# aleflabo/PREGO

Measured on AMD Instinct MI355X. Metric: frames/sec (per-frame action logits) on Assembly101-O TSN features, higher is better.
Workload: dtype fp16; 1 GPU; BASELINE configs[1]: Assembly101-O-test-split-shaped eval set, MiniROAD eval path (rgb+flow fp32 [T,2048] each -> per-frame probs[86] + argmax); clips_per_gpu=182, frames_per_gpu=2306143, min_T=3342, max_T=33981, flow=non-zero (full K=4096 layer1 GEMM), parallelism=clip-sharded dp1, no collective: every rank its own eval-set-sized clip list, weights=random init, seed 20

## Files before the change

### include/prego_amd_debug.h

```cpp
#ifndef PREGO_AMD_DEBUG_H
#define PREGO_AMD_DEBUG_H
#include "prego_amd.h"
#ifdef __cplusplus
extern "C" {
#endif

int prego_debug_head_only(prego_miniroad* h, int n_slots, int n_steps, const void* h_relu, float* out, int32_t* argmax,
                          const void* rowmap , prego_stream_t stream);

int prego_miniroad_debug_stamps(prego_miniroad* h, unsigned long long* out8);

int prego_debug_recurrence_only(prego_miniroad* h, int n_slots, int n_steps, int gd, const void* gi, void* h_relu, prego_stream_t stream);
int prego_debug_gemm_worker(const void* A, const void* B, const float* bias, float* C, int M, int N, int K, int xcd_lo,
                            unsigned* counter, int grid, prego_stream_t stream);

int prego_debug_split_fault(prego_miniroad* h, int mode);
int prego_debug_split_state(const prego_miniroad* h, int64_t* fallbacks, int32_t* fails, int64_t* skip, int32_t* split_env);
int prego_debug_set_abort(prego_miniroad* h, unsigned value, prego_stream_t stream);
int prego_debug_alloc_count(int64_t* device_mallocs, int64_t* host_waits);
int prego_debug_ant_full_span(int on);
int prego_debug_hog(int kind, int xcd_lo, int ms, const void* read_buf, void* write_buf, size_t bytes, float* sink, prego_stream_t stream);

int prego_debug_gemm_bf16(int variant, const void* A, const void* B, const float* bias, float* C, int M, int N, int K,
                          prego_stream_t stream);

int prego_debug_gemm_tn(int ta, int tb, const void* A, int lda, const void* B, int ldb, const float* bias, float* C, void* C16, int ldc,
                        int M, int N, int K, int k_valid, float* colsum_out, prego_stream_t stream);

int prego_debug_gemm_nt(int f16, int train_splitk, const void* A, int lda, const void* B, int ldb, const float* bias, float* C, int ldc,
                        int M, int N, int K, prego_stream_t stream);

int prego_debug_attention_bwd(int batch, int len, int heads, int dh, int causal, const void* qs, const void* k, const void* v,
                              const void* o, const void* dout, const float* lse, void* dqkv, prego_stream_t stream);

int prego_debug_attention_fwd(int batch, int n_query, int len, int heads, int dh, int causal, const void* qs, const void* k,
                              const void* v, void* out, float* lse, prego_stream_t stream);

#ifdef __cplusplus
}
#endif
#endif
```

### prego_amd/_lib.py

```python
from __future__ import annotations

import ctypes as C
import os

_HERE = os.path.dirname(os.path.abspath(__file__))
DEBUG_LIB_PATH = os.path.join(_HERE, "lib", "libprego_amd_debug.so")
LIB_PATH = os.environ.get("PREGO_AMD_LIB") or (DEBUG_LIB_PATH if os.environ.get("PREGO_AMD_DEBUG_LIB") else os.path.join(_HERE, "lib", "libprego_amd.so"))

PREGO_F32, PREGO_BF16, PREGO_F16, PREGO_F16X2 = 0, 1, 2, 3
FWD_SOFTMAX, FWD_KEEP, FWD_IN16 = 1, 2, 4
E_TIMEOUT = -4

SYMBOLS = [
    "prego_abi_version", "prego_last_error",
    "prego_miniroad_create", "prego_miniroad_create_layers", "prego_miniroad_set_gru_layer", "prego_miniroad_destroy", "prego_miniroad_last_error", "prego_miniroad_set_weights",
    "prego_miniroad_max_clips", "prego_miniroad_workspace_bytes", "prego_miniroad_forward",
    "prego_miniroad_check", "prego_miniroad_timing_enable", "prego_miniroad_timing_read",
    "prego_miniroad_set_dropout", "prego_oad_loss", "prego_oad_loss_reduce",
    "prego_miniroad_backward_workspace_bytes", "prego_miniroad_backward", "prego_adamw_step", "prego_miniroad_adamw_step", "prego_window_vote", "prego_format_ids", "prego_perframe_ap_labels", "prego_onehot_labels",
    "prego_vit_create", "prego_vit_destroy", "prego_vit_num_tensors", "prego_vit_set_weights",
    "prego_vit_workspace_bytes", "prego_vit_forward",
    "prego_vit_set_dropout", "prego_vit_train_workspace_bytes", "prego_vit_forward_train", "prego_vit_backward",
    "prego_attention_layer_workspace_bytes", "prego_attention_layer_forward",
    "prego_attention_layer_create", "prego_attention_layer_destroy", "prego_attention_layer_set_weights",
    "prego_attention_layer_handle_workspace_bytes", "prego_attention_layer_handle_forward",
    "prego_attention_layer_set_dropout", "prego_attention_layer_train_workspace_bytes", "prego_attention_layer_forward_train", "prego_attention_layer_backward", "prego_vit_adamw_step", "prego_miniroad_step",
    "prego_perframe_ap_workspace_bytes", "prego_perframe_ap", "prego_vit_frames_workspace_bytes", "prego_vit_forward_frames", "prego_miniroad_backward_events", "prego_miniroad_backward_callback",
    "prego_miniroad_plan_starts", "prego_miniroad_set_feed_events", "prego_miniroad_pass_info",
    "prego_vit_set_compute_dtype", "prego_attention_layer_set_compute_dtype",
    "prego_miniroad_resident_bytes", "prego_miniroad_set_resident", "prego_miniroad_guard_publish", "prego_miniroad_set_peer_guard",
    "prego_miniroad_set_gru_layer_grads",
    "prego_miniroad_set_anticipation", "prego_miniroad_forward_anticipation",
    "prego_miniroad_set_anticipation_grads", "prego_miniroad_adamw_step_anticipation",
    "prego_miniroad_step_anticipation",
    "prego_miniroad_step_wide_workspace_bytes", "prego_miniroad_step_wide", "prego_miniroad_step_wide_anticipation",
    "prego_cast_features",
    "prego_stream_pool_bytes", "prego_stream_pool_create", "prego_stream_pool_destroy", "prego_miniroad_step_pool_workspace_bytes",
    "prego_miniroad_step_pool", "prego_stream_pool_vote", "prego_stream_pool_flush", "prego_stream_pool_reset", "prego_stream_pool_record",
    "prego_miniroad_step_frames_workspace_bytes", "prego_miniroad_step_frames", "prego_miniroad_step_frames_anticipation",
    "prego_miniroad_step_pool_frames_workspace_bytes", "prego_miniroad_step_pool_frames",
    "prego_miniroad_step_ragged_workspace_bytes", "prego_miniroad_step_ragged", "prego_miniroad_step_ragged_anticipation",
    "prego_miniroad_step_pool_ragged_workspace_bytes", "prego_miniroad_step_pool_ragged",
]
DEBUG_SYMBOLS = ["prego_miniroad_debug_stamps", "prego_debug_gemm_bf16", "prego_debug_attention_bwd", "prego_debug_attention_fwd",
                 "prego_debug_recurrence_only", "prego_debug_gemm_worker", "prego_debug_head_only",
                 "prego_debug_split_fault", "prego_debug_split_state", "prego_debug_set_abort", "prego_debug_alloc_count", "prego_debug_hog",
                 "prego_debug_ant_full_span", "prego_debug_gemm_tn", "prego_debug_gemm_nt"]


class PregoError(RuntimeError):
    pass


_lib = None


def _open(path: str, debug: bool) -> C.CDLL:
    if not os.path.exists(path):
        raise PregoError(
            f"{path} not found: the HIP library has not been built. Run `python -m prego_amd.build` "
            "(needs hipcc; cross-compiles gfx950 without a GPU). There is no CPU fallback.")
    import torch
    lib = C.CDLL(path)
    vp, i32, i64, sz = C.c_void_p, C.c_int, C.c_int64, C.c_size_t
    lib.prego_abi_version.restype = i32
    lib.prego_last_error.restype = C.c_char_p
    lib.prego_miniroad_create.argtypes = [C.POINTER(vp), i32, i32, i32, i32, i32, i32]
    lib.prego_miniroad_create_layers.argtypes = [C.POINTER(vp), i32, i32, i32, i32, i32, i32, i32]
    lib.prego_miniroad_set_gru_layer.argtypes = [vp, i32, vp, vp, vp, vp, vp]
    lib.prego_miniroad_destroy.argtypes = [vp]
    lib.prego_miniroad_destroy.restype = None
    lib.prego_miniroad_last_error.argtypes = [vp]
    lib.prego_miniroad_last_error.restype = C.c_char_p
    lib.prego_miniroad_set_weights.argtypes = [vp] + [vp] * 10 + [vp]
    lib.prego_miniroad_max_clips.argtypes = [vp]
    lib.prego_miniroad_workspace_bytes.argtypes = [vp, i32, C.POINTER(C.c_int32), i64, i32]
    lib.prego_miniroad_workspace_bytes.restype = sz
    lib.prego_miniroad_resident_bytes.argtypes = [vp, i32, C.POINTER(C.c_int32), i32]
    lib.prego_miniroad_resident_bytes.restype = sz
    lib.prego_miniroad_set_resident.argtypes = [vp, vp, sz]
    lib.prego_miniroad_guard_publish.argtypes = [vp, vp, vp]
    lib.prego_miniroad_set_peer_guard.argtypes = [vp, vp]
    lib.prego_miniroad_set_gru_layer_grads.argtypes = [vp, i32, vp, vp, vp, vp]
    lib.prego_miniroad_forward.argtypes = [vp, i32, C.POINTER(C.c_int32), C.POINTER(vp), C.POINTER(vp),
                                           C.POINTER(vp), C.POINTER(vp), vp, vp, i32, vp, sz, vp]
    lib.prego_miniroad_set_anticipation.argtypes = [vp, i32, vp, vp, vp]
    lib.prego_miniroad_forward_anticipation.argtypes = [vp, i32, C.POINTER(C.c_int32), C.POINTER(vp), C.POINTER(vp),
                                                        C.POINTER(vp), C.POINTER(vp), C.POINTER(vp), C.POINTER(vp), vp, vp, i32, vp, sz, vp]
    lib.prego_miniroad_set_anticipation_grads.argtypes = [vp, C.POINTER(vp), vp, vp]
    lib.prego_miniroad_step.argtypes = [vp, i32, vp, vp, vp, vp, vp, i32, vp]
    lib.prego_miniroad_step_anticipation.argtypes = [vp, i32, vp, vp, vp, vp, vp, vp, vp, i32, vp]
    lib.prego_miniroad_step_wide_workspace_bytes.argtypes = [vp, i32]
    lib.prego_miniroad_step_wide_workspace_bytes.restype = sz
    lib.prego_miniroad_step_wide.argtypes = [vp, i32, vp, vp, vp, vp, vp, i32, vp, sz, vp]
    lib.prego_miniroad_step_wide_anticipation.argtypes = [vp, i32, vp, vp, vp, vp, vp, vp, vp, i32, vp, sz, vp]
    lib.prego_stream_pool_bytes.argtypes = [vp, i32, i32]
    lib.prego_stream_pool_bytes.restype = sz
    lib.prego_stream_pool_create.argtypes = [C.POINTER(vp), vp, i32, i32, i32, vp, sz, vp]
    lib.prego_stream_pool_destroy.argtypes = [vp]
    lib.prego_stream_pool_destroy.restype = None
    lib.prego_miniroad_step_pool_workspace_bytes.argtypes = [vp, i32]
    lib.prego_miniroad_step_pool_workspace_bytes.restype = sz
    lib.prego_miniroad_step_pool.argtypes = [vp, vp, i32, C.POINTER(C.c_int32), vp, vp, vp, vp, vp, vp, i32, vp, sz, vp]
    lib.prego_miniroad_step_frames_workspace_bytes.argtypes = [vp, i32, i32]
    lib.prego_miniroad_step_frames_workspace_bytes.restype = sz
    lib.prego_miniroad_step_frames.argtypes = [vp, i32, i32, vp, vp, vp, vp, vp, i32, vp, sz, vp]
    lib.prego_miniroad_step_frames_anticipation.argtypes = [vp, i32, i32, vp, vp, vp, vp, vp, vp, vp, i32, vp, sz, vp]
    lib.prego_miniroad_step_pool_frames_workspace_bytes.argtypes = [vp, i32, i32]
    lib.prego_miniroad_step_pool_frames_workspace_bytes.restype = sz
    lib.prego_miniroad_step_pool_frames.argtypes = [vp, vp, i32, i32, C.POINTER(C.c_int32), vp, vp, vp, vp, vp, vp, i32, vp, sz, vp]
    lib.prego_miniroad_step_ragged_workspace_bytes.argtypes = [vp, i32, i32]
    lib.prego_miniroad_step_ragged_workspace_bytes.restype = sz
    lib.prego_miniroad_step_ragged.argtypes = [vp, i32, C.POINTER(C.c_int32), vp, vp, vp, vp, vp, i32, vp, sz, vp]
    lib.prego_miniroad_step_ragged_anticipation.argtypes = [vp, i32, C.POINTER(C.c_int32), vp, vp, vp, vp, vp, vp, vp, i32, vp, sz, vp]
    lib.prego_miniroad_step_pool_ragged_workspace_bytes.argtypes = [vp, i32, i32]
    lib.prego_miniroad_step_pool_ragged_workspace_bytes.restype = sz
    lib.prego_miniroad_step_pool_ragged.argtypes = [vp, vp, i32, C.POINTER(C.c_int32), C.POINTER(C.c_int32), vp, vp, vp, vp, vp, vp, i32, vp, sz,
                                                    vp]
    lib.prego_stream_pool_vote.argtypes = [vp, i32, C.POINTER(C.c_int32), vp, vp]
    lib.prego_stream_pool_flush.argtypes = [vp, i32, C.POINTER(C.c_int32), vp]
    lib.prego_stream_pool_reset.argtypes = [vp, i32, C.POINTER(C.c_int32), vp]
    lib.prego_stream_pool_record.argtypes = [vp, i32, C.POINTER(vp), C.POINTER(sz)]
    lib.prego_miniroad_check.argtypes = [vp, vp]
    lib.prego_miniroad_timing_enable.argtypes = [vp, i32]
    lib.prego_miniroad_timing_read.argtypes = [vp, C.POINTER(C.c_double), C.POINTER(i64), C.POINTER(C.c_double),
                                               C.POINTER(C.c_double), C.POINTER(i64), C.POINTER(C.c_double),
                                               C.POINTER(i64), C.POINTER(C.c_double)]
    lib.prego_miniroad_set_dropout.argtypes = [vp, C.c_float, C.c_uint64]
    lib.prego_oad_loss.argtypes = [i32, C.POINTER(C.c_int32), C.POINTER(vp), C.POINTER(vp), i32, vp, C.POINTER(vp),
                                   C.c_float, vp]
    lib.prego_oad_loss_reduce.argtypes = [i32, C.POINTER(C.c_int32), C.POINTER(vp), C.POINTER(vp), i32, i32, vp, C.POINTER(vp),
                                          C.c_float, vp]
    lib.prego_miniroad_backward_workspace_bytes.argtypes = [vp, i32, C.POINTER(C.c_int32)]
    lib.prego_miniroad_backward_workspace_bytes.restype = sz
    lib.prego_miniroad_backward.argtypes = [vp, i32, C.POINTER(C.c_int32), C.POINTER(vp)] + [vp] * 10 + [vp, sz, vp, sz, vp]
    lib.prego_miniroad_backward_events.argtypes = [vp, vp, vp]
    lib.prego_miniroad_backward_callback.argtypes = [vp, vp, vp]
    lib.prego_miniroad_plan_starts.argtypes = [vp, i32, C.POINTER(C.c_int32), i32, C.POINTER(C.c_int32), C.POINTER(C.c_int32)]
    lib.prego_miniroad_set_feed_events.argtypes = [vp, i32, C.POINTER(C.c_int32), C.POINTER(vp), i32]
    lib.prego_miniroad_pass_info.argtypes = [vp, C.POINTER(C.c_int32), C.POINTER(C.c_int32), C.POINTER(C.c_int32)]
    lib.prego_window_vote.argtypes = [vp, i64, i32, i32, vp, vp]
    lib.prego_format_ids.argtypes = [vp, i64, vp, vp, vp]
    lib.prego_cast_features.argtypes = [vp, vp, i64, i32, vp]
    lib.prego_perframe_ap_workspace_bytes.argtypes = [i64, i32]
    lib.prego_perframe_ap_workspace_bytes.restype = sz
    lib.prego_perframe_ap.argtypes = [vp, vp, i64, i32, vp, vp, vp, vp, sz, vp]
    lib.prego_perframe_ap_labels.argtypes = [vp, vp, i64, i32, vp, vp, vp, vp, sz, vp]
    lib.prego_onehot_labels.argtypes = [i32, C.POINTER(vp), C.POINTER(i64), i32, vp, C.POINTER(C.c_int32)]
    f32 = C.c_float
    lib.prego_adamw_step.argtypes = [i32, C.POINTER(vp), C.POINTER(vp), C.POINTER(vp), C.POINTER(vp), C.POINTER(i64), i64, f32, f32, f32, f32, f32, vp]
    lib.prego_miniroad_adamw_step.argtypes = [vp, C.POINTER(vp), C.POINTER(vp), C.POINTER(vp), C.POINTER(vp), i64, f32, f32, f32, f32, f32, vp]
    lib.prego_miniroad_adamw_step_anticipation.argtypes = [vp, C.POINTER(vp), C.POINTER(vp), C.POINTER(vp), C.POINTER(vp), i64, f32, f32, f32, f32, f32, vp]
    lib.prego_vit_adamw_step.argtypes = [vp, C.POINTER(vp), C.POINTER(vp), C.POINTER(vp), C.POINTER(vp), i32, i64, f32, f32, f32, f32, f32, vp]
    lib.prego_vit_create.argtypes = [C.POINTER(vp)] + [i32] * 8
    lib.prego_vit_destroy.argtypes = [vp]
    lib.prego_vit_destroy.restype = None
    lib.prego_vit_num_tensors.argtypes = [vp]
    lib.prego_vit_set_weights.argtypes = [vp, C.POINTER(vp), i32, vp]
    lib.prego_vit_workspace_bytes.argtypes = [vp, i32]
    lib.prego_vit_workspace_bytes.restype = sz
    lib.prego_vit_forward.argtypes = [vp, i32, vp, vp, vp, i32, vp, sz, vp]
    lib.prego_vit_frames_workspace_bytes.argtypes = [vp, i32, i32]
    lib.prego_vit_frames_workspace_bytes.restype = sz
    lib.prego_vit_forward_frames.argtypes = [vp, i32, vp, vp, vp, vp, i32, i32, vp, sz, vp]
    lib.prego_vit_set_compute_dtype.argtypes = [vp, i32]
    lib.prego_attention_layer_set_compute_dtype.argtypes = [vp, i32]
    lib.prego_vit_set_dropout.argtypes = [vp, C.c_float, C.c_float, C.c_uint64]
    lib.prego_vit_train_workspace_bytes.argtypes = [vp, i32]
    lib.prego_vit_train_workspace_bytes.restype = sz
    lib.prego_vit_forward_train.argtypes = [vp, i32, vp, vp, vp, i32, vp, sz, vp]
    lib.prego_vit_backward.argtypes = [vp, i32, vp, C.POINTER(vp), i32, i32, vp, sz, vp]
    lib.prego_attention_layer_workspace_bytes.argtypes = [i32, i32, i32]
    lib.prego_attention_layer_workspace_bytes.restype = sz
    lib.prego_attention_layer_forward.argtypes = [i32] * 5 + [vp] * 10 + [vp, sz, vp]
    lib.prego_attention_layer_create.argtypes = [C.POINTER(vp), i32, i32]
    lib.prego_attention_layer_destroy.argtypes = [vp]
    lib.prego_attention_layer_destroy.restype = None
    lib.prego_attention_layer_set_weights.argtypes = [vp] + [vp] * 8 + [vp]
    lib.prego_attention_layer_handle_workspace_bytes.argtypes = [vp, i32, i32]
    lib.prego_attention_layer_handle_workspace_bytes.restype = sz
    lib.prego_attention_layer_handle_forward.argtypes = [vp, i32, i32, i32, vp, vp, vp, sz, vp]
    lib.prego_attention_layer_set_dropout.argtypes = [vp, C.c_float, C.c_uint64]
    lib.prego_attention_layer_train_workspace_bytes.argtypes = [vp, i32, i32]
    lib.prego_attention_layer_train_workspace_bytes.restype = sz
    lib.prego_attention_layer_forward_train.argtypes = [vp, i32, i32, i32, vp, vp, vp, sz, vp]
    lib.prego_attention_layer_backward.argtypes = [vp, i32, i32, i32, vp, vp, vp, i32, vp, sz, vp]
    for name in SYMBOLS:
        getattr(lib, name)
    if debug:
        lib.prego_miniroad_debug_stamps.argtypes = [vp, C.POINTER(C.c_uint64)]
        lib.prego_debug_head_only.argtypes = [vp, i32, i32, vp, vp, vp, vp, vp]
        lib.prego_debug_attention_bwd.argtypes = [i32] * 5 + [vp] * 7 + [vp]
        lib.prego_debug_attention_fwd.argtypes = [i32] * 6 + [vp] * 5 + [vp]
        lib.prego_debug_recurrence_only.argtypes = [vp, i32, i32, i32, vp, vp, vp]
        lib.prego_debug_gemm_worker.argtypes = [vp, vp, vp, vp, i32, i32, i32, i32, vp, i32, vp]
        lib.prego_debug_gemm_bf16.argtypes = [i32, vp, vp, vp, vp, i32, i32, i32, vp]
        lib.prego_debug_gemm_tn.argtypes = [i32, i32, vp, i32, vp, i32, vp, vp, vp, i32, i32, i32, i32, i32, vp, vp]
        lib.prego_debug_gemm_nt.argtypes = [i32, i32, vp, i32, vp, i32, vp, vp, i32, i32, i32, i32, vp]
        lib.prego_debug_split_fault.argtypes = [vp, i32]
        lib.prego_debug_split_state.argtypes = [vp, C.POINTER(i64), C.POINTER(i32), C.POINTER(i64), C.POINTER(i32)]
        lib.prego_debug_set_abort.argtypes = [vp, C.c_uint32, vp]
        lib.prego_debug_alloc_count.argtypes = [C.POINTER(i64), C.POINTER(i64)]
        lib.prego_debug_hog.argtypes = [i32, i32, i32, vp, vp, sz, vp, vp]
        lib.prego_debug_ant_full_span.argtypes = [i32]
    return lib


def load() -> C.CDLL:
    global _lib
    if _lib is None:
        _lib = _open(LIB_PATH, debug=LIB_PATH == DEBUG_LIB_PATH)
    return _lib


_dbg = None


def load_debug() -> C.CDLL:
    global _dbg
    if _dbg is None:
        _dbg = load() if LIB_PATH == DEBUG_LIB_PATH else _open(DEBUG_LIB_PATH, debug=True)
    return _dbg




def check(rc: int):
    if rc != 0:
        raise PregoError(f"prego_amd error {rc}: {load().prego_last_error().decode()}")


def ptr_array(ptrs):
    arr = (C.c_void_p * len(ptrs))()
    for i, p in enumerate(ptrs):
        arr[i] = p
    return arr
```

### prego_amd/csrc/ff_pass.hip

```cpp
#include "common.h"
#include "kernels.h"
#include "pass_handshake.h"

#define FBK 64
#define FHALF 16384
#define FBUF 65536
#define FF_WAIT(n) asm volatile("s_waitcnt vmcnt(" #n ")" ::: "memory")
#define FF_TIMEOUT_TICKS 200000000ull

__device__ __forceinline__ int ffp_key_b(int r) { return ((r >> 1) & 1) | (((r >> 3) & 3) << 1); }

__device__ __forceinline__ bool ffp_wait_ge(const unsigned* p, unsigned need, unsigned* abort_word, unsigned code) {
  if (__hip_atomic_load(p, __ATOMIC_RELAXED, __HIP_MEMORY_SCOPE_AGENT) >= need) return true;
  const unsigned long long t0 = __builtin_amdgcn_s_memrealtime();
  unsigned spins = 0;
  for (;;) {
    __builtin_amdgcn_s_sleep(8);
    if (__hip_atomic_load(p, __ATOMIC_RELAXED, __HIP_MEMORY_SCOPE_AGENT) >= need) return true;
    if ((++spins & 31u) == 0u) {
      if (__hip_atomic_load(abort_word, __ATOMIC_RELAXED, __HIP_MEMORY_SCOPE_AGENT)) return false;
      if (__builtin_amdgcn_s_memrealtime() - t0 > FF_TIMEOUT_TICKS) {
        __hip_atomic_store(abort_word, code, __ATOMIC_RELAXED, __HIP_MEMORY_SCOPE_AGENT);
        return false;
      }
    }
  }
}

template <typename OT, bool SC1OUT>
__device__ __forceinline__ void ffp_tile(char* smem, const bf16_t* __restrict__ A, int lda, int rows, const bf16_t* __restrict__ B, int ldb,
                                         const float* __restrict__ bias, bf16_t* __restrict__ C, int ldc, int K) {
  int tid = threadIdx.x;
  asm volatile("" : "+v"(tid));
  const int lane = tid & 63;
  const int wave = __builtin_amdgcn_readfirstlane(tid >> 6);
  const int grp = wave >> 2, wc = wave & 3;
  const int nk = K / FBK;
  const int sr = lane >> 3, scp = lane & 7;
  int a_off[2], b_off[2];
#pragma unroll
  for (int i = 0; i < 2; ++i) {
    const int r = (wave * 2 + i) * 8 + sr;
    a_off[i] = r * lda * 2 + ((scp ^ ((r >> 1) & 7)) << 4);
    b_off[i] = r * ldb * 2 + ((scp ^ ffp_key_b(r)) << 4);
  }
  const __amdgpu_buffer_rsrc_t rs_a = __builtin_amdgcn_make_buffer_rsrc((void*)A, 0, rows * lda * 2, 0x00020000);
  const __amdgpu_buffer_rsrc_t rs_b = __builtin_amdgcn_make_buffer_rsrc((void*)B, 0, 256 * ldb * 2, 0x00020000);
  auto stage_a = [&](int hf, int kt) {
    char* dst = smem + (kt & 1) * FBUF + hf * FHALF + wave * 2048;
    const int so = hf * 128 * lda * 2 + kt * (FBK * 2);
#pragma unroll
    for (int i = 0; i < 2; ++i)
      __builtin_amdgcn_raw_ptr_buffer_load_lds(rs_a, (__attribute__((address_space(3))) void*)(dst + i * 1024), 16, a_off[i], so, 0, 0);
  };
  auto stage_b = [&](int hf, int kt) {
    char* dst = smem + (kt & 1) * FBUF + (2 + hf) * FHALF + wave * 2048;
    const int so = hf * 128 * ldb * 2 + kt * (FBK * 2);
#pragma unroll
    for (int i = 0; i < 2; ++i)
      __builtin_amdgcn_raw_ptr_buffer_load_lds(rs_b, (__attribute__((address_space(3))) void*)(dst + i * 1024), 16, b_off[i], so, 0, 0);
  };
  const int fr = lane & 15, fq = lane >> 4;
  bf16x8 a0[2][4], a1[2][4], b0[2][2], b1[2][2];
  auto read_a = [&](bf16x8 (&af)[2][4], int slot, int kt) {
    const char* base = smem + (kt & 1) * FBUF + slot * FHALF;
#pragma unroll
    for (int ks = 0; ks < 2; ++ks)
#pragma unroll
      for (int i = 0; i < 4; ++i) {
        const int r = grp * 64 + i * 16 + fr;
        af[ks][i] = *(const bf16x8*)(base + r * 128 + (((ks * 4 + fq) ^ ((r >> 1) & 7)) << 4));
      }
  };
  auto read_b = [&](bf16x8 (&bf)[2][2], int slot, int kt) {
    const char* base = smem + (kt & 1) * FBUF + slot * FHALF;
#pragma unroll
    for (int ks = 0; ks < 2; ++ks)
#pragma unroll
      for (int j = 0; j < 2; ++j) {
        const int r = wc * 32 + (fr >> 2) * 8 + j * 4 + (fr & 3);
        bf[ks][j] = *(const bf16x8*)(base + r * 128 + (((ks * 4 + fq) ^ ffp_key_b(r)) << 4));
      }
  };
  f32x4 acc[2][2][4][2];
#pragma unroll
  for (int x = 0; x < 2; ++x)
#pragma unroll
    for (int y = 0; y < 2; ++y)
#pragma unroll
      for (int i = 0; i < 4; ++i)
#pragma unroll
        for (int j = 0; j < 2; ++j) acc[x][y][i][j] = (f32x4){0.f, 0.f, 0.f, 0.f};
  auto mma = [&](f32x4 (&c)[4][2], const bf16x8 (&af)[2][4], const bf16x8 (&bf)[2][2]) {
    asm volatile("s_waitcnt lgkmcnt(0)" ::: "memory");
    __builtin_amdgcn_sched_barrier(0);
    __builtin_amdgcn_s_setprio(1);
#pragma unroll
    for (int ks = 0; ks < 2; ++ks)
#pragma unroll
      for (int i = 0; i < 4; ++i)
#pragma unroll
        for (int j = 0; j < 2; ++j) c[i][j] = op16<OT>::mfma(bf[ks][j], af[ks][i], c[i][j]);
    __builtin_amdgcn_s_setprio(0);
    __builtin_amdgcn_sched_barrier(0);
  };
  auto bar = [&]() {
    __builtin_amdgcn_sched_barrier(0);
    __builtin_amdgcn_s_barrier();
    __builtin_amdgcn_sched_barrier(0);
  };
  stage_a(0, 0); stage_b(0, 0); stage_b(1, 0); stage_a(1, 0);
  stage_a(0, 1); stage_b(0, 1); stage_b(1, 1);
  FF_WAIT(10);
  bar();
  read_a(a0, 0, 0);
  if (grp == 1) bar();
  for (int kt = 0; kt < nk; ++kt) {
    const bool full = kt + 2 < nk;
    read_b(b0, 2, kt);
    if (kt + 1 < nk) stage_a(1, kt + 1);
    if (full) FF_WAIT(10); else FF_WAIT(0);
    bar();
    mma(acc[0][0], a0, b0);
    bar();
    read_b(b1, 3, kt);
    if (full) { stage_a(0, kt + 2); FF_WAIT(10); } else FF_WAIT(0);
    bar();
    mma(acc[0][1], a0, b1);
    bar();
    read_a(a1, 1, kt);
    if (full) { stage_b(0, kt + 2); FF_WAIT(10); } else FF_WAIT(0);
    bar();
    mma(acc[1][1], a1, b1);
    bar();
    if (kt + 1 < nk) read_a(a0, 0, kt + 1);
    if (full) { stage_b(1, kt + 2); FF_WAIT(10); } else FF_WAIT(0);
    bar();
    mma(acc[1][0], a1, b0);
    bar();
  }
  if (grp == 0) bar();
  float4 bv[2][2];
#pragma unroll
  for (int y = 0; y < 2; ++y)
#pragma unroll
    for (int j = 0; j < 2; ++j) bv[y][j] = *(const float4*)(bias + y * 128 + wc * 32 + fq * 8 + j * 4);
  const __amdgpu_buffer_rsrc_t rs_c = __builtin_amdgcn_make_buffer_rsrc((void*)C, 0, rows * ldc * 2, 0x00020000);
#pragma unroll
  for (int x = 0; x < 2; ++x)
#pragma unroll
    for (int y = 0; y < 2; ++y) {
      const int n = y * 128 + wc * 32 + fq * 8;
#pragma unroll
      for (int i = 0; i < 4; ++i) {
        const int m = x * 128 + grp * 64 + i * 16 + fr;
        const f32x4 v0 = acc[x][y][i][0], v1 = acc[x][y][i][1];
        u32x4 pk;
        pk[0] = op16<OT>::pack2_sat(v0[0] + bv[y][0].x, v0[1] + bv[y][0].y); pk[1] = op16<OT>::pack2_sat(v0[2] + bv[y][0].z, v0[3] + bv[y][0].w);
        pk[2] = op16<OT>::pack2_sat(v1[0] + bv[y][1].x, v1[1] + bv[y][1].y); pk[3] = op16<OT>::pack2_sat(v1[2] + bv[y][1].z, v1[3] + bv[y][1].w);
        if constexpr (SC1OUT) __builtin_amdgcn_raw_buffer_store_b128(pk, rs_c, (m * ldc + n) * 2, 0, AUX_SC1);
        else __builtin_amdgcn_raw_buffer_store_b128(pk, rs_c, (m * ldc + n) * 2, 0, 0);
      }
    }
}

template <typename OT, bool IN16>
__device__ __forceinline__ void ffp_pack_rows(const FfPassArgs& a, int my_rows, int wave, int lane, const char* srgb, const char* sflow,
                                              bf16_t* __restrict__ Xs) {
  constexpr int ES = IN16 ? 2 : 4, NV = IN16 ? 1 : 2;
  constexpr int PR = 2;
  const int din = a.kx;
  const int cr_rgb = (a.d_rgb + 2047) >> 11, cpr = cr_rgb + ((a.d_flow + 2047) >> 11);
  const int n_rounds = my_rows > 0 ? ((my_rows + PR - 1) / PR) * cpr : 0;
  auto readlane_ptr = [](const char* p, int l) -> const char* {
    const unsigned long long v = (unsigned long long)p;
    const unsigned lo = (unsigned)__builtin_amdgcn_readlane((int)(unsigned)v, l), hi = (unsigned)__builtin_amdgcn_readlane((int)(unsigned)(v >> 32), l);
    return (const char*)(((unsigned long long)hi << 32) | lo);
  };
  int voff_in = lane * 8 * ES, voff_in2 = voff_in + 1024 * ES, voff_out = lane * 16;
  asm volatile("" : "+v"(voff_in), "+v"(voff_in2), "+v"(voff_out));
  auto issue = [&](u32x4 (&v)[PR][4][NV], int k) {
    const int rp = k / cpr, cj = k - rp * cpr;
    const bool fl = cj >= cr_rgb;
    const int cwin = (fl ? cj - cr_rgb : cj) << 11, seg_len = fl ? a.d_flow : a.d_rgb;
#pragma unroll
    for (int e = 0; e < PR; ++e) {
      const int r = rp * PR + e, rr = r < my_rows ? r : 0;
      const char* s0 = readlane_ptr(srgb, rr);
      const char* s1 = readlane_ptr(sflow, rr);
      const char* src = fl ? s1 : s0;
      const __amdgpu_buffer_rsrc_t rs = __builtin_amdgcn_make_buffer_rsrc((void*)(src + (size_t)cwin * ES), 0,
                                                                          (r < my_rows && src != nullptr) ? (seg_len - cwin) * ES : 0, 0x00020000);
#pragma unroll
      for (int b = 0; b < 4; ++b)
#pragma unroll
        for (int w = 0; w < NV; ++w)
          v[e][b][w] = __builtin_amdgcn_raw_buffer_load_b128(rs, (b < 2 ? voff_in : voff_in2) + ((b & 1) * 512 * ES + 16 * w), 0, AUX_NT);
    }
  };
  auto drain = [&](const u32x4 (&v)[PR][4][NV], int k) {
    const int rp = k / cpr, cj = k - rp * cpr;
    const bool fl = cj >= cr_rgb;
    const int cwin = (fl ? cj - cr_rgb : cj) << 11, seg_len = fl ? a.d_flow : a.d_rgb, seg_base = fl ? a.d_rgb : 0;
#pragma unroll
    for (int e = 0; e < PR; ++e) {
      const int r = rp * PR + e;
      bf16_t* dst = Xs + (size_t)(wave * 32 + (r < my_rows ? r : 0)) * din + seg_base + cwin;
      const __amdgpu_buffer_rsrc_t rs = __builtin_amdgcn_make_buffer_rsrc((void*)dst, 0, r < my_rows ? (seg_len - cwin) * 2 : 0, 0x00020000);
#pragma unroll
      for (int b = 0; b < 4; ++b) {
        u32x4 o = v[e][b][0];
        if constexpr (!IN16) {
          const u32x4 x = v[e][b][0], y = v[e][b][NV - 1];
          o[0] = op16<OT>::pack2_sat(__uint_as_float(x[0]), __uint_as_float(x[1])); o[1] = op16<OT>::pack2_sat(__uint_as_float(x[2]), __uint_as_float(x[3]));
          o[2] = op16<OT>::pack2_sat(__uint_as_float(y[0]), __uint_as_float(y[1])); o[3] = op16<OT>::pack2_sat(__uint_as_float(y[2]), __uint_as_float(y[3]));
        }
        __builtin_amdgcn_raw_buffer_store_b128(o, rs, voff_out + b * 1024, 0, 0);
      }
    }
  };
  u32x4 va[PR][4][NV], vb[PR][4][NV];
  if (n_rounds == 0) return;
  issue(va, 0);
  int k = 0;
#define PACK_FENCE() __builtin_amdgcn_sched_barrier(0)
  for (; k + 2 < n_rounds; k += 2) {
    issue(vb, k + 1); PACK_FENCE();
    drain(va, k); PACK_FENCE();
    issue(va, k + 2); PACK_FENCE();
    drain(vb, k + 1); PACK_FENCE();
  }
  if (k + 1 < n_rounds) {
    issue(vb, k + 1); PACK_FENCE();
    drain(va, k); PACK_FENCE();
    drain(vb, k + 1);
  } else {
    drain(va, k);
  }
#undef PACK_FENCE
}

template <typename OT>
__device__ __forceinline__ void ffp_pack(const FfPassArgs& a, int row0, int nrows, bf16_t* __restrict__ Xs) {
  int tid_ = threadIdx.x;
  asm volatile("" : "+v"(tid_));
  const int lane = tid_ & 63, wave = __builtin_amdgcn_readfirstlane(tid_ >> 6);
  const int rl = wave * 32 + (lane & 31);
  int clip = 0, t = 0;
  if (rl < nrows) {
    const int row = row0 + rl;
    int lo = a.plan.blk_step[row >> 5];
    while (lo + 1 < a.plan.s_max && a.plan.rowoff[lo + 1] <= row) ++lo;
    const int slot = row - a.plan.rowoff[lo];
    int k = a.plan.seg_off[slot];
    const int kend = a.plan.seg_off[slot + 1];
    while (k + 1 < kend && a.plan.seg_start[k + 1] <= lo) ++k;
    clip = a.plan.seg_clip[k];
    t = lo - a.plan.seg_start[k];
    if (a.rowmap != nullptr && lane < 32) ((int2*)a.rowmap)[row] = make_int2(clip, t);
  }
  const char* srgb = nullptr; const char* sflow = nullptr;
  const int es = a.in16 ? 2 : 4;
  if (rl < nrows) {
    const float* rgb = a.rgb_ptrs ? a.rgb_ptrs[clip] : nullptr;
    const float* flow = a.flow_ptrs ? a.flow_ptrs[clip] : nullptr;
    if (rgb) srgb = (const char*)rgb + (size_t)t * a.d_rgb * es;
    if (flow) sflow = (const char*)flow + (size_t)t * a.d_flow * es;
  }
  const int my_rows = nrows - wave * 32 < 32 ? nrows - wave * 32 : 32;
  if (a.in16) ffp_pack_rows<OT, true>(a, my_rows, wave, lane, srgb, sflow, Xs);
  else ffp_pack_rows<OT, false>(a, my_rows, wave, lane, srgb, sflow, Xs);
}

constexpr int FLN_MAX_E = 2048;

template <typename OT, int NV, int NR>
__device__ __forceinline__ void ffp_ln(const FfPassArgs& a, int nrows, const bf16_t* __restrict__ Ys, bf16_t* __restrict__ Es, const float* gb) {
  int tid_ = threadIdx.x;
  asm volatile("" : "+v"(tid_));
  const int lane = tid_ & 63, wave = __builtin_amdgcn_readfirstlane(tid_ >> 6);
  const int E = NV * 512;
  const float fE = (float)a.E;
  if (wave >= nrows) return;
  auto request = [&](u32x4 (&dst)[NR][NV], int rb) {
#pragma unroll
    for (int e = 0; e < NR; ++e) {
      int r = rb + 8 * e;
      if (r >= nrows) r = wave;
      const bf16_t* y = Ys + (size_t)r * E;
#pragma unroll
      for (int i = 0; i < NV; ++i) dst[e][i] = *(const u32x4*)(y + (i * 64 + lane) * 8);
    }
  };
  auto unpack = [](const u32x4 w, float (&f)[8]) {
    f[0] = op16<OT>::lo(w[0]); f[1] = op16<OT>::hi(w[0]); f[2] = op16<OT>::lo(w[1]); f[3] = op16<OT>::hi(w[1]);
    f[4] = op16<OT>::lo(w[2]); f[5] = op16<OT>::hi(w[2]); f[6] = op16<OT>::lo(w[3]); f[7] = op16<OT>::hi(w[3]);
  };
  auto process = [&](const u32x4 (&raw)[NR][NV], int rb) {
    float s[NR];
#pragma unroll
    for (int e = 0; e < NR; ++e) {
      s[e] = 0.f;
#pragma unroll
      for (int i = 0; i < NV; ++i) {
        float f[8];
        unpack(raw[e][i], f);
        s[e] += ((f[0] + f[1]) + (f[2] + f[3])) + ((f[4] + f[5]) + (f[6] + f[7]));
      }
    }
    auto wave_sum_rows = [](float (&v)[NR]) {
#pragma unroll
      for (int o = 32; o > 0; o >>= 1) {
        float t[NR];
#pragma unroll
        for (int e = 0; e < NR; ++e) t[e] = __shfl_xor(v[e], o, 64);
#pragma unroll
        for (int e = 0; e < NR; ++e) v[e] += t[e];
      }
    };
    float mu[NR], rstd[NR];
    wave_sum_rows(s);
#pragma unroll
    for (int e = 0; e < NR; ++e) mu[e] = s[e] / fE;
#pragma unroll
    for (int e = 0; e < NR; ++e) {
      float qq = 0.f;
#pragma unroll
      for (int i = 0; i < NV; ++i) {
        float f[8];
        unpack(raw[e][i], f);
#pragma unroll
        for (int k = 0; k < 8; ++k) {
#pragma clang fp contract(off)
          const float d = f[k] - mu[e];
          const float dd = d * d;
          qq = qq + dd;
        }
      }
      rstd[e] = qq;
    }
    wave_sum_rows(rstd);
#pragma unroll
    for (int e = 0; e < NR; ++e) rstd[e] = 1.0f / sqrtf(rstd[e] / fE + a.ln_eps);
#pragma unroll
    for (int i = 0; i < NV; ++i) {
      const int c = (i * 64 + lane) * 8;
      const float4 g0 = *(const float4*)(gb + c), g1 = *(const float4*)(gb + c + 4);
      const float4 b0 = *(const float4*)(gb + FLN_MAX_E + c), b1 = *(const float4*)(gb + FLN_MAX_E + c + 4);
      const float gg[8] = {g0.x, g0.y, g0.z, g0.w, g1.x, g1.y, g1.z, g1.w};
      const float bb[8] = {b0.x, b0.y, b0.z, b0.w, b1.x, b1.y, b1.z, b1.w};
#pragma unroll
      for (int e = 0; e < NR; ++e) {
        float f[8], o[8];
        unpack(raw[e][i], f);
#pragma unroll
        for (int k = 0; k < 8; ++k) o[k] = fmaxf((f[k] - mu[e]) * rstd[e] * gg[k] + bb[k], 0.f);
        uint4 w;
        w.x = op16<OT>::pack2_sat(o[0], o[1]); w.y = op16<OT>::pack2_sat(o[2], o[3]); w.z = op16<OT>::pack2_sat(o[4], o[5]); w.w = op16<OT>::pack2_sat(o[6], o[7]);
        if (rb + 8 * e < nrows) *(uint4*)(Es + (size_t)(rb + 8 * e) * E + c) = w;
      }
    }
  };
  constexpr int STEP = 8 * NR;
#define LN_FENCE() __builtin_amdgcn_sched_barrier(0)
  u32x4 ra[NR][NV], rbuf[NR][NV];
  int rb = wave;
  request(ra, rb); LN_FENCE();
  for (; rb + 2 * STEP < nrows; rb += 2 * STEP) {
    request(rbuf, rb + STEP); LN_FENCE();
    process(ra, rb); LN_FENCE();
    request(ra, rb + 2 * STEP); LN_FENCE();
    process(rbuf, rb + STEP); LN_FENCE();
  }
  if (rb + STEP < nrows) {
    request(rbuf, rb + STEP); LN_FENCE();
    process(ra, rb); LN_FENCE();
    process(rbuf, rb + STEP);
  } else {
    process(ra, rb);
  }
#undef LN_FENCE
}

template <typename OT, int MAXV, int NR>
__device__ __forceinline__ void ffp_ln_generic(const FfPassArgs& a, int nrows, const bf16_t* __restrict__ Ys, bf16_t* __restrict__ Es) {
  int tid_ = threadIdx.x;
  asm volatile("" : "+v"(tid_));
  const int lane = tid_ & 63, wave = tid_ >> 6;
  const int E = a.E, nv = E / 512;
  u32x4 raw[NR][MAXV], nxt[NR][MAXV];
  auto request = [&](u32x4 (&dst)[NR][MAXV], int rb) {
#pragma unroll
    for (int e = 0; e < NR; ++e) {
      int r = rb + 8 * e;
      if (r >= nrows) r = wave < nrows ? wave : 0;
      const bf16_t* y = Ys + (size_t)r * E;
#pragma unroll
      for (int i = 0; i < MAXV; ++i)
        if (i < nv) dst[e][i] = *(const u32x4*)(y + (i * 64 + lane) * 8);
    }
  };
  if (wave < nrows) request(raw, wave);
  for (int rb = wave; rb < nrows; rb += 8 * NR) {
    if (rb + 8 * NR < nrows) request(nxt, rb + 8 * NR);
    auto unpack = [](const u32x4 w, float (&f)[8]) {
      f[0] = op16<OT>::lo(w[0]); f[1] = op16<OT>::hi(w[0]); f[2] = op16<OT>::lo(w[1]); f[3] = op16<OT>::hi(w[1]);
      f[4] = op16<OT>::lo(w[2]); f[5] = op16<OT>::hi(w[2]); f[6] = op16<OT>::lo(w[3]); f[7] = op16<OT>::hi(w[3]);
    };
    float s[NR];
#pragma unroll
    for (int e = 0; e < NR; ++e) {
      s[e] = 0.f;
#pragma unroll
      for (int i = 0; i < MAXV; ++i)
        if (i < nv) {
          float f[8];
          unpack(raw[e][i], f);
          s[e] += ((f[0] + f[1]) + (f[2] + f[3])) + ((f[4] + f[5]) + (f[6] + f[7]));
        }
    }
    float mu[NR], rstd[NR];
#pragma unroll
    for (int e = 0; e < NR; ++e) mu[e] = wave_sum(s[e]) / (float)E;
#pragma unroll
    for (int e = 0; e < NR; ++e) {
      float qq = 0.f;
#pragma unroll
      for (int i = 0; i < MAXV; ++i)
        if (i < nv) {
          float f[8];
          unpack(raw[e][i], f);
#pragma unroll
          for (int k = 0; k < 8; ++k) {
#pragma clang fp contract(off)
            const float d = f[k] - mu[e];
            const float dd = d * d;
            qq = qq + dd;
          }
        }
      rstd[e] = qq;
    }
#pragma unroll
    for (int e = 0; e < NR; ++e) rstd[e] = 1.0f / sqrtf(wave_sum(rstd[e]) / (float)E + a.ln_eps);
#pragma unroll
    for (int i = 0; i < MAXV; ++i)
      if (i < nv) {
        const int c = (i * 64 + lane) * 8;
        const float4 g0 = *(const float4*)(a.ln_g + c), g1 = *(const float4*)(a.ln_g + c + 4);
        const float4 b0 = *(const float4*)(a.ln_b + c), b1 = *(const float4*)(a.ln_b + c + 4);
        const float gg[8] = {g0.x, g0.y, g0.z, g0.w, g1.x, g1.y, g1.z, g1.w};
        const float bb[8] = {b0.x, b0.y, b0.z, b0.w, b1.x, b1.y, b1.z, b1.w};
#pragma unroll
        for (int e = 0; e < NR; ++e) {
          float f[8], o[8];
          unpack(raw[e][i], f);
#pragma unroll
          for (int k = 0; k < 8; ++k) o[k] = fmaxf((f[k] - mu[e]) * rstd[e] * gg[k] + bb[k], 0.f);
          uint4 w;
          w.x = op16<OT>::pack2_sat(o[0], o[1]); w.y = op16<OT>::pack2_sat(o[2], o[3]); w.z = op16<OT>::pack2_sat(o[4], o[5]); w.w = op16<OT>::pack2_sat(o[6], o[7]);
          if (rb + 8 * e < nrows) *(uint4*)(Es + (size_t)(rb + 8 * e) * E + c) = w;
        }
      }
    if (rb + 8 * NR < nrows) {
#pragma unroll
      for (int e = 0; e < NR; ++e)
#pragma unroll
        for (int i = 0; i < MAXV; ++i)
          if (i < nv) raw[e][i] = nxt[e][i];
    }
  }
}

template <typename OT>
__device__ __forceinline__ void ffp_ln_any(const FfPassArgs& a, int nrows, const bf16_t* __restrict__ Ys, bf16_t* __restrict__ Es, const float* gb) {
  switch (a.E >> 9) {
    case 4: ffp_ln<OT, 4, 2>(a, nrows, Ys, Es, gb); break;
    case 2: ffp_ln<OT, 2, 4>(a, nrows, Ys, Es, gb); break;
    case 1: ffp_ln<OT, 1, 4>(a, nrows, Ys, Es, gb); break;
    default: ffp_ln_generic<OT, 8, 2>(a, nrows, Ys, Es); break;
  }
}

template <typename OT>
__global__ __launch_bounds__(512, 2) void ff_pass_kernel(FfPassArgs a) {
  extern __shared__ __attribute__((aligned(16))) char smem[];
  __shared__ int s_job[2];
  const int tid = threadIdx.x;
  const int xcc = __builtin_amdgcn_readfirstlane(__builtin_amdgcn_s_getreg((3 << 11) | 20) & 7);
  if (xcc < a.xcd_lo) return;
  if (tid == 0) {
    const unsigned nth = __hip_atomic_fetch_add(a.hs.ff_here + xcc, 1u, __ATOMIC_RELAXED, __HIP_MEMORY_SCOPE_AGENT);
    s_job[1] = hs_wait(a.hs, a.hs.ticks_all) == PREGO_HS_GO ? 1 : 0;
    if (a.max_wg > 0 && (int)nth >= a.max_wg) s_job[1] = 0;
  }
  __syncthreads();
  if (!__builtin_amdgcn_readfirstlane(s_job[1])) return;
  __shared__ __attribute__((aligned(16))) float s_gb[2 * FLN_MAX_E];
  if (a.E <= FLN_MAX_E)
    for (int c = tid; c < a.E; c += 512) { s_gb[c] = a.ln_g[c]; s_gb[FLN_MAX_E + c] = a.ln_b[c]; }
  const int q = xcc - a.xcd_lo, nf = 8 - a.xcd_lo;
  const int n_q = a.n_units > q ? (a.n_units - q + nf - 1) / nf : 0;
  const int sg = a.sg, tpr = sg * (2 + a.nt1 + a.nt2);
  const int n_rounds = (n_q + sg - 1) / sg + a.lag3;
  __shared__ unsigned long long s_stat[11];
  const bool stats = a.stats != nullptr && tid == 0;
  if (stats) {
    for (int e = 0; e < 8; ++e) s_stat[e] = 0;
    s_stat[9] = __builtin_amdgcn_s_memrealtime(); s_stat[8] = s_stat[9]; s_stat[10] = __builtin_amdgcn_s_memtime();
  }
#define FSTAT(i) do { if (stats) { const unsigned long long n_ = __builtin_amdgcn_s_memrealtime(); s_stat[i] += n_ - s_stat[8]; s_stat[8] = n_; } } while (0)
  for (;;) {
    __syncthreads();
    if (tid == 0) s_job[0] = (int)__hip_atomic_fetch_add(a.tick + q, 1u, __ATOMIC_RELAXED, __HIP_MEMORY_SCOPE_AGENT);
    __syncthreads();
    const int k = __builtin_amdgcn_readfirstlane(s_job[0]);
    const int round = k / tpr, j = k - round * tpr;
    FSTAT(5);
    if (round >= n_rounds) break;
    int type, i, nb = 0;
    if (j < sg) { type = 0; i = round * sg + j; }
    else if (j < sg + sg * a.nt1) { const int jj = j - sg; type = 1; nb = jj / sg; i = (round - a.lag1) * sg + (jj - nb * sg); }
    else if (j < 2 * sg + sg * a.nt1) { type = 2; i = (round - a.lag2) * sg + (j - sg - sg * a.nt1); }
    else { const int jj = j - 2 * sg - sg * a.nt1; type = 3; nb = jj / sg; i = (round - a.lag3) * sg + (jj - nb * sg); }
    if (i < 0 || i >= n_q) continue;
    const int u = q + i * nf;
    if (tid == 0) {
      bool ok = true;
      const int up = u - a.ring_units;
      if (type == 0) {
        if (up >= 0) ok = ffp_wait_ge(a.l1_cnt + up, (unsigned)a.nt1, a.abort_word, 0x100u);
      } else if (type == 1) {
        ok = ffp_wait_ge(a.pack_done + u, 1u, a.abort_word, 0x101u);
        if (ok && up >= 0) ok = ffp_wait_ge(a.ln_done + up, 1u, a.abort_word, 0x102u);
      } else if (type == 2) {
        ok = ffp_wait_ge(a.l1_cnt + u, (unsigned)a.nt1, a.abort_word, 0x103u);
        if (ok && up >= 0) ok = ffp_wait_ge(a.wih_cnt + up, (unsigned)a.nt2, a.abort_word, 0x104u);
      } else {
        ok = ffp_wait_ge(a.ln_done + u, 1u, a.abort_word, 0x105u);
        const int ug = u - a.gi_ring_units;
        if (ok && ug >= 0) ok = ffp_wait_ge(a.rec_cnt + (ug >> a.chunk_unit_shift), (unsigned)a.rec_expect, a.abort_word, 0x106u);
      }
      s_job[1] = ok ? 1 : 0;
    }
    __syncthreads();
    if (!__builtin_amdgcn_readfirstlane(s_job[1])) break;
    FSTAT(4);
    asm volatile("buffer_inv sc0" ::: "memory");
    const int row0 = u * 256;
    const int nrows = a.total_rows - row0 < 256 ? a.total_rows - row0 : 256;
    const size_t slot = (size_t)(u % a.ring_units) * 256;
    if (type == 0) {
      if (!(a.dbg & 1)) ffp_pack<OT>(a, row0, nrows, a.X + slot * a.kx);
    } else if (type == 1) {
      if (!(a.dbg & 4))
      ffp_tile<OT, false>(smem, a.X + slot * a.kx, a.kx, nrows, a.w1 + (size_t)nb * 256 * a.ld_w1, a.ld_w1, a.b1 + nb * 256,
                          a.Y + slot * a.E + nb * 256, a.E, a.kx);
    } else if (type == 2) {
      if (a.dbg & 2) { }
      else ffp_ln_any<OT>(a, nrows, a.Y + slot * a.E, a.Eb + slot * a.E, s_gb);
    } else {
      const size_t gslot = (size_t)(u & (a.gi_ring_units - 1)) * 256;
      if (!(a.dbg & 8))
      ffp_tile<OT, true>(smem, a.Eb + slot * a.E, a.E, nrows, a.w_ih + (size_t)nb * 256 * a.E, a.E, a.bias2 + nb * 256,
                         a.GI + gslot * a.n3 + nb * 256, a.n3, a.E);
    }
    asm volatile("s_waitcnt vmcnt(0)" ::: "memory");
    __syncthreads();
    FSTAT(type);
    if (tid == 0) {
      if (type == 0) __hip_atomic_store(a.pack_done + u, 1u, __ATOMIC_RELAXED, __HIP_MEMORY_SCOPE_AGENT);
      else if (type == 1) __hip_atomic_fetch_add(a.l1_cnt + u, 1u, __ATOMIC_RELAXED, __HIP_MEMORY_SCOPE_AGENT);
      else if (type == 2) __hip_atomic_store(a.ln_done + u, 1u, __ATOMIC_RELAXED, __HIP_MEMORY_SCOPE_AGENT);
      else {
        const unsigned old = __hip_atomic_fetch_add(a.wih_cnt + u, 1u, __ATOMIC_RELAXED, __HIP_MEMORY_SCOPE_AGENT);
        if (old + 1u == (unsigned)a.nt2)
          __hip_atomic_fetch_add(a.gi_cnt + (u >> a.chunk_unit_shift), 1u, __ATOMIC_RELAXED, __HIP_MEMORY_SCOPE_AGENT);
      }
    }
  }
  if (stats) {
    s_stat[7] = __builtin_amdgcn_s_memrealtime() - s_stat[9];
    s_stat[6] = __builtin_amdgcn_s_memtime() - s_stat[10];
    for (int e = 0; e < 8; ++e) atomicAdd(a.stats + e, s_stat[e]);
  }
#undef FSTAT
}

int launch_ff_pass(const FfPassArgs& a, hipStream_t s) {
  if (a.E % 512 || a.E > 4096 || a.kx % FBK || a.kx < 2 * FBK || a.n3 % 256 || a.xcd_lo < 1 || a.xcd_lo > 7) return -1;
  if (a.sg < 1 || a.ring_units % (8 - a.xcd_lo) || (a.gi_ring_units & (a.gi_ring_units - 1)) || a.nt1 != a.E / 256 || a.nt2 != a.n3 / 256) return -1;
  static DeviceOnce once;
  once.run([&] {
    (void)hipFuncSetAttribute((const void*)ff_pass_kernel<bf16_t>, hipFuncAttributeMaxDynamicSharedMemorySize, 2 * FBUF);
    (void)hipFuncSetAttribute((const void*)ff_pass_kernel<f16_t>, hipFuncAttributeMaxDynamicSharedMemorySize, 2 * FBUF);
  });
  if (a.f16) ff_pass_kernel<f16_t><<<256, 512, 2 * FBUF, s>>>(a);
  else ff_pass_kernel<bf16_t><<<256, 512, 2 * FBUF, s>>>(a);
  return 0;
}
```

### prego_amd/csrc/kernels.h

```cpp
#pragma once
#include <hip/hip_runtime_api.h>
#include <stddef.h>
#include <stdint.h>
#include <mutex>

const char* prego_tune_env(const char* name);

struct DeviceOnce {
  std::mutex mu;
  bool done[64] = {};
  template <class F> int run(F&& f) {
    int dev = 0;
    (void)hipGetDevice(&dev);
    if (dev < 0 || dev >= 64) { f(); return 0; }
    std::lock_guard<std::mutex> g(mu);
    if (!done[dev]) { f(); done[dev] = true; }
    return dev;
  }
};

#ifndef PREGO_HAVE_SLOTPLAN
struct SlotPlan {
  const int* rowoff; const int* nact; const int* seg_off; const int* seg_clip; const int* seg_start; const int* blk_step;
  int s_max; int n_slots;
};
#define PREGO_HAVE_SLOTPLAN 1
#endif

struct PassHandshake {
  unsigned* word;
  unsigned* ff_here;
  unsigned* host;
  unsigned seq;
  unsigned ticks_lead;
  unsigned ticks_all;
};
#define PREGO_HS_GO 1u
#define PREGO_HS_FAIL 2u

struct GruArgs {
  const void* whh;
  const float* b_hn;
  const void* gi;
  void* h_relu_out;
  float* h_raw_out;
  float* h_state;
  void* hx;
  unsigned* flags;
  unsigned* abort_word;
  const int* rowoff;
  const int* nact;
  int t0, t1;
  int row_base;
  int n_clips;
  int G;
  const int* seg_off; const int* seg_start;
  float* keep_r; float* keep_z; float* keep_n; float* keep_ghn;
  unsigned* sync;
  unsigned long long* stamps;
  int gi_bf16;
  int f16;
  int Gd;
  int rows;
  int armed;
  int no_mt;
  const unsigned* gi_cnt;
  unsigned* rec_cnt;
  int chunk_shift, n_chunks;
  int units_per_chunk, units_last;
  unsigned gi_row_mask;
  PassHandshake hs;
  float out_floor;
};
struct FfPassArgs {
  const float* const* rgb_ptrs; const float* const* flow_ptrs;
  SlotPlan plan;
  void* rowmap;
  int d_rgb, d_flow;
  int in16;
  int kx;
  const unsigned short* w1; int ld_w1; const float* b1;
  const float* ln_g; const float* ln_b; float ln_eps;
  const unsigned short* w_ih; const float* bias2;
  int E, n3;
  unsigned short* X; unsigned short* Y; unsigned short* Eb;
  unsigned short* GI;
  int ring_units, gi_ring_units;
  int total_rows, n_units;
  int xcd_lo;
  int chunk_unit_shift;
  int rec_expect;
  int nt1, nt2;
  int sg;
  int max_wg;
  int lag1, lag2, lag3;
  int dbg;
  unsigned long long* stats;
  int f16;
  unsigned* tick;
  unsigned* pack_done; unsigned* l1_cnt; unsigned* ln_done; unsigned* wih_cnt;
  unsigned* gi_cnt;
  const unsigned* rec_cnt;
  unsigned* abort_word;
  PassHandshake hs;
};
int launch_ff_pass(const FfPassArgs& a, hipStream_t s);
int launch_gru_recurrence_pass(int hid, GruArgs a, hipStream_t s);
int gru_group_size(bool bf16, int hid);
bool gru_hidden_supported(bool bf16, int hid);
void launch_gru_arm(bool bf16, int hid, int G, void* hx, unsigned* sync, hipStream_t s);

struct GruArm { unsigned* hx; unsigned long long words_per_buf; unsigned pattern; unsigned* sync; };
GruArm gru_arm_desc(bool bf16, int hid, int G, void* hx, unsigned* sync);

struct BpttArgs {
  const void* whhT;
  const float* dHout;
  const float* R; const float* Z; const float* N; const float* GHN;
  const float* Hraw;
  float* dGI; float* dGH;
  void* dGIop; void* dGHop;
  void* hx;
  unsigned* sync;
  unsigned* abort_word;
  const int* rowoff; const int* nact;
  int t_max, n_clips, G;
  int force_sc1;
};
size_t gru_bptt_hx_bytes(bool bf16, int hid, int G);
int launch_gru_bptt(bool bf16, int hid, int nct, BpttArgs a, hipStream_t s);

enum { EPI_STORE = 0, EPI_RESIDUAL = 1, EPI_GELU_BF16 = 2, EPI_STORE_BF16 = 3, EPI_QKV = 4, EPI_TOKENS = 5 };
struct GemmEpi {
  int mode;
  void* out_b;
  void* q; void* k;
  int n_tok, heads, dh, emb;
  float q_scale;
  void* vn;
  int which0;
  unsigned drop_thresh; float drop_scale; unsigned long long drop_seed;
  unsigned drop2_thresh; float drop2_scale; unsigned long long drop2_seed;
  float* pre_f32;
  const float* pe;
  int f16;
  int xcd_lo; unsigned* counter;
  int split_a_lo, split_b_lo;
  const float* acc_scale;
};
void launch_gemm_bf16_nt_epi(const void* A, int lda, const void* B, int ldb, const float* bias, float* C, int ldc, int M,
                             int N, int K, GemmEpi epi, hipStream_t s);

void launch_pack_rows(bool bf16, const float* const* rgb_ptrs, const float* const* flow_ptrs, const SlotPlan& plan,
                      int row0, int nrows, int d_rgb, int d_flow, void* X, hipStream_t s, int grid_limit = 0,
                      void* rowmap = nullptr ,
                      bool f16 = false ,
                      bool in16 = false );
void launch_ln_relu(bool bf16, const void* Y, const float* gamma, const float* beta, int nrows, int E, float eps,
                    void* out, float* stats, float drop_p, unsigned long long seed, int row0_abs, hipStream_t s, int relu = 1,
                    bool in_bf16 = false, bool f16 = false, const GruArm* arm = nullptr);
void launch_f32_to_bf16(const float* src, void* dst, size_t n, hipStream_t s);
void launch_pad_convert(bool bf16, const float* src, int rows_src, int cols_src, int ld_src, void* dst, int rows_dst,
                        int cols_dst, hipStream_t s, bool f16 = false);
int launch_gemm_bf16_pingpong_mode(int mode, const void* A, int lda, const void* B, int ldb, const float* bias, void* C, int ldc,
                                   int M, int N, int K, bool out_bf16, hipStream_t s, bool f16 = false);
int launch_gemm_bf16_pingpong_epi(const void* A, int lda, const void* B, int ldb, const float* bias, void* C, int ldc, int M, int N,
                                  int K, GemmEpi epi, hipStream_t s);
int launch_gemm_bf16_pingpong_worker(const void* A, int lda, const void* B, int ldb, const float* bias, void* C, int ldc, int M, int N,
                                     int K, int xcd_lo, unsigned* counter, int grid, hipStream_t s, bool out16 = false, bool f16 = false);
int launch_gemm_x2_pingpong(const void* A, int lda, int a_lo, const void* B, int ldb, int b_lo, const float* inv_scale, const float* bias,
                            float* C, int ldc, int M, int N, int K, hipStream_t s);
void launch_x2_weight_split(const float* src, int rows, int cols, void* dst, float* scale2 , hipStream_t s);
void launch_pack_rows_x2(const float* const* rgb_ptrs, const float* const* flow_ptrs, const SlotPlan& plan, int row0, int nrows,
                         int d_rgb, int d_flow, void* X, hipStream_t s, int grid_limit = 0, void* rowmap = nullptr);
void launch_ln_relu_x2(const float* Y, const float* gamma, const float* beta, int nrows, int E, float eps, void* out, hipStream_t s,
                       const GruArm* arm = nullptr);
int launch_gru_recurrence_x2(int hid, int nct, GruArgs a, const float* inv_scale, hipStream_t s);
size_t gru_x2_hx_bytes(int hid, int G);
GruArm gru_x2_arm_desc(int hid, int G, void* hx, unsigned* sync);
int launch_gemm_bf16_pingpong(const void* A, int lda, const void* B, int ldb, const float* bias, float* C, int ldc, int M, int N,
                              int K, hipStream_t s);
void launch_gemm_bf16_nt(const void* A, int lda, const void* B, int ldb, const float* bias, float* C, int ldc, int M,
                         int N, int K, hipStream_t s, bool f16 = false,
                         bool train_splitk = false );
void launch_gemm_f32_nt(const float* A, int lda, const float* B, int ldb, const float* bias, float* C, int ldc, int M,
                        int N, int K, hipStream_t s);
int launch_gru_recurrence(bool bf16, int hid, int nct, GruArgs a, hipStream_t s);
size_t gru_hx_bytes(bool bf16, int hid, int G);
int gru_max_tiles();
int launch_head_softmax(bool bf16, const void* Hrelu, const void* Wc, const float* bc, const SlotPlan& plan,
                        int row0, int nrows, int hid, int C, int apply_softmax,
                        float* const* out_ptrs, int* const* argmax_ptrs, hipStream_t s, const void* rowmap = nullptr, bool f16 = false);
int launch_ant_head(bool bf16, bool f16, const void* Hrelu, const void* Wa, const float* ba, const void* Wc, const float* bc,
                    const SlotPlan& plan, int row0, int nrows, int hid, int L, int C, int apply_softmax, float* const* out_ptrs,
                    int* const* argmax_ptrs, const void* rowmap, hipStream_t s);
int launch_ant_head_store_a(bool bf16, const void* Hrelu, const void* Wa, const float* ba, int nrows, int hid, int L, void* a_out,
                            const int* span, hipStream_t s);
void launch_ant_gather(const float* const* d_ant, const int* rowoff, const int* sorted_clip, int t_max, int nrows, int LC, float* G, int* flags,
                       int* span, int force_full, hipStream_t s);
void launch_ant_head_wgrad(bool bf16, const float* G, const void* HR, const void* Wc, int R, int H, int L, int C, const int* span,
                           const void* Abuf, void* dZ, float* g_fc_w, float* g_fc_b, float* g_w_a, float* g_b_a, hipStream_t s);
void launch_ant_head_dgrad(bool bf16, const void* Wa, int R, int H, int L, const int* span, const void* dZ, float* part, float* dHR, hipStream_t s);
void launch_permute_rows(const float* src, float* dst, const int* sorted_clip, int n, int width, int to_sorted,
                         hipStream_t s);
void launch_add_vec(const float* a, const float* b, float* out, int n, int n_add, hipStream_t s);

void launch_oad_loss(const float* const* logit_ptrs, const float* const* target_ptrs, const int* lens, int n_clips, int C,
                     float* loss_out, float* const* dlogit_ptrs, float grad_scale, hipStream_t s, bool sum = false);
void launch_gather_dlogits(bool bf16, const float* const* dl_ptrs, const int* rowoff, const int* sorted_clip, int t_max,
                           int nrows, int C, int Cpad, void* out, hipStream_t s);
void launch_transpose_convert(bool in_bf16, bool out_bf16, const void* src, int M, int N, int ld_src, void* dst, int Mpad,
                              hipStream_t s);
void launch_colsum(const float* src, int M, int N, float* part, float* out, hipStream_t s);
void launch_colsum_bf16(const void* src, int M, int N, float* part, float* out, hipStream_t s);
void launch_colsum_stage2(const float* part, int nb, int N, float* out, hipStream_t s);
void launch_gru_bwd_step(bool bf16, int t, int na, int na_next, int row_t, int row_tm1, int H, const float* dHout,
                         const float* carry_in, const float* dhpart, const float* R, const float* Z, const float* Nn,
                         const float* GHN, const float* Hraw, float* carry_out, float* dGI, float* dGH, void* dGIop,
                         void* dGHop, hipStream_t s);
void launch_relu_mask(const float* dHrelu, const float* Hraw, size_t n, float* out, hipStream_t s);
void launch_build_hprev(bool bf16, const float* Hraw, const int* rowoff, int t_max, int nrows, int H, void* out,
                        hipStream_t s);
int launch_ln_relu_bwd(const float* dE, const float* Y, const float* stats, const float* gamma, const float* beta, int nrows,
                       int E, float drop_p, unsigned long long seed, int row0_abs, float* dY, float* part, hipStream_t s,
                       int relu = 1, int accumulate = 0, void* dYb = nullptr );
int launch_gemm_bf16_tn(bool ta, bool tb, const void* A, int lda, const void* B, int ldb, const float* bias, float* C, int ldc, int M, int N,
                        int K, int k_valid, float* colsum_out, hipStream_t s, void* C16 = nullptr );

int launch_window_vote(const int* pred, long long n_frames, int window, int n_classes, int* votes, hipStream_t s);

int launch_format_ids(const int* ids, long long n, unsigned* text, int* bad, hipStream_t s);
size_t perframe_ap_workspace_bytes(long long n_frames, int n_classes);
int launch_perframe_ap(const float* scores, const float* target, const int* labels, long long n_frames, int n_classes, double* ap, long long* n_pos,
                       double* score_sum, void* workspace, hipStream_t s);

void launch_cast_features(bool f16, const float* src, void* dst, long long n, int n_cu, hipStream_t s);

constexpr int kPoolMaxActive = 256;
constexpr int kPoolRecHeader = 4;
constexpr int kPoolOverflowFull = 1, kPoolOverflowBadId = 2;
struct PoolGeom {
  float* h;
  int* rec;
  int hid, ncls, ncls_pad, window, max_events, rec_words, capacity;
};
struct PoolSlots { int s[kPoolMaxActive]; };
int launch_pool_gather(const PoolGeom& g, const int* slots, int n, float* h_ws, hipStream_t s);
int launch_pool_commit(const PoolGeom& g, const int* slots, int n, const float* h_ws, const int* argmax, hipStream_t s);
int launch_pool_commit_frames(const PoolGeom& g, const int* slots, int n, int K, const float* h_ws, const int* argmax, hipStream_t s);
int launch_pool_vote(const PoolGeom& g, const int* slots, int n, const int* ids, hipStream_t s);
int launch_pool_flush(const PoolGeom& g, const int* slots, int n, hipStream_t s);
int launch_pool_reset(const PoolGeom& g, const int* slots, int n, hipStream_t s);

void launch_permute_gi_rows(const void* w, const float* bias, void* w_perm, float* bias_perm, int H, int E, hipStream_t s);

int launch_adamw(int n_tensors, float* const* params, const float* const* grads, float* const* exp_avg, float* const* exp_avg_sq,
                 void* const* copies, const long long* numel, bool copy_bf16, long long step, float lr, float b1, float b2, float eps,
                 float wd, hipStream_t s, unsigned* guard = nullptr ,
                 const float* peer = nullptr );

int launch_flash_attention_v2(const void* Q, const void* K, const void* V, void* out, int B, int Nq, int N, int heads, int dh,
                              int causal, hipStream_t s, float* lse = nullptr, unsigned drop_thresh = 0, float drop_scale = 1.f,
                              unsigned long long drop_seed = 0, bool f16 = false );
int launch_attention_bwd(const void* Qs, const void* K, const void* V, const void* O, const void* dO, const float* lse,
                         float* delta, void* dqkv, int B, int N, int heads, int dh, int causal, float q_scale, hipStream_t s,
                         unsigned drop_thresh = 0, float drop_scale = 1.f, unsigned long long drop_seed = 0);
void launch_gelu_bwd(const float* df, const float* u, size_t n, float* du, void* du_bf16, hipStream_t s, unsigned drop_thresh = 0,
                     float drop_scale = 1.f, unsigned long long drop_seed = 0);
void launch_mask_convert(const float* src, size_t n, float* out_f32, void* out_bf16, unsigned drop_thresh, float drop_scale,
                         unsigned long long drop_seed, hipStream_t s, unsigned drop2_thresh = 0, float drop2_scale = 1.f,
                         unsigned long long drop2_seed = 0);
void launch_vit_head_bwd(const float* x, const float* dlogits, int B, int N, int E, int C, const float* lnw, const float* lnb,
                         const float* hw, float* dx, float* scratch , float* g_lnw, float* g_lnb, float* g_hw,
                         float* g_hb, hipStream_t s);
void launch_vit_tokens_bwd(const float* dx, int B, int T, int E, float* denc, float* g_pe, float* g_cls, hipStream_t s,
                           unsigned drop_thresh = 0, float drop_scale = 1.f, unsigned long long drop_seed = 0);
void launch_cat_convert(const float* rgb, const float* flow, int rows, int d_rgb, int d_flow, void* out_bf16, hipStream_t s, bool f16 = false);
void launch_vit_tokens(const float* enc, const float* cls, const float* pe, int B, int T, int E, float* x, hipStream_t s,
                       unsigned drop_thresh = 0, float drop_scale = 1.f, unsigned long long drop_seed = 0);
void launch_vit_cls_rows(const float* cls, const float* pe, int B, int T, int E, float* x, hipStream_t s);
void launch_vit_head(const float* x, int B, int N, int E, const float* lnw, const float* lnb, const float* hw,
                     const float* hb, int C, float* out, hipStream_t s, int* argmax = nullptr);
void launch_vit_sliding_tokens(const float* enc, const float* enc_b, const float* cls, const float* pe, int t0, int B, int T, int E,
                               float* x, const float* ln_w, const float* ln_b, void* xn, float* x0, hipStream_t s, bool f16 = false);
void launch_add_bias_rows(float* x, const float* bias, int rows, int n, hipStream_t s);
int launch_attention_f32(const float* qkv, int ld, int q_off, int k_off, int v_off, float* out, int B, int N, int Nq, int heads,
                         int dh, int causal, float scale, hipStream_t s);
void launch_gelu_f32(float* u, size_t n, hipStream_t s);
void launch_add_rows(float* x, const float* y, size_t n, hipStream_t s);
void launch_cat_rows_f32(const float* rgb, const float* flow, int rows, int d_rgb, int d_flow, float* out, hipStream_t s);

struct StreamGemv {
  const void* W;
  const void* X;
  const void* X2;
  const float* bias;
  float* Y;
  int Nout, K, kx1, ldx, ldx2, x_bf16;
  const float* ln_g = nullptr;
  const float* ln_b = nullptr;
  float ln_eps = 1e-5f;
};
int launch_stream_gemv(int nprob, const StreamGemv* pr, int n, hipStream_t s, bool f16 = false);
int launch_stream_gates_head(const float* gi, const float* gh, const float* b_hn, float* h_state, const void* wc, const float* bc, int n,
                              int H, int C, int softmax, float* out, int* argmax, hipStream_t s, bool f16 = false);

int launch_stream_ant_hidden(const void* wa, const float* ba, const float* h_state, void* A, int n, int H, int L, hipStream_t s, bool f16 = false);
int launch_stream_ant_head(const void* A, const void* wc, const float* bc, int n, int H, int L, int C, int softmax, float* ant_out,
                           int* ant_argmax, hipStream_t s, bool f16 = false);

int launch_wide_cast(const float* rgb, const float* flow, const float* h_state, void* xb, void* hb, int n, int d_rgb, int d_flow, int H,
                     hipStream_t s, bool f16 = false);
int launch_wide_gemv(int nprob, const StreamGemv* pr, int n, hipStream_t s, bool f16 = false);
int launch_wide_ant_hidden(const void* wa, const float* ba, const float* h_state, void* A, int n, int H, int L, hipStream_t s, bool f16 = false);
int launch_wide_ant_head(const void* A, const void* wc, const float* bc, int n, int H, int L, int C, int softmax, float* ant_out,
                         int* ant_argmax, hipStream_t s, bool f16 = false);

int launch_frames_cast(const float* rgb, const float* flow, const float* h_state, void* xb, float* h0, int rows, int n, int d_rgb, int d_flow,
                       int H, hipStream_t s, bool f16 = false);
int launch_frames_recur(const void* whh, const float* gi, const float* b_hn, const float* h0, float* hist, void* hr, float* h_state, int n,
                        int K, int t, int H, hipStream_t s, bool f16 = false);

constexpr int kRaggedMaxStreams = 256;
struct RaggedMap { unsigned e[kRaggedMaxStreams]; };
__host__ __device__ inline unsigned ragged_entry(unsigned off, unsigned stream, unsigned count) { return off | (stream << 16) | (count << 24); }
__host__ __device__ inline unsigned ragged_off(unsigned e) { return e & 0xffffu; }
__host__ __device__ inline unsigned ragged_stream(unsigned e) { return (e >> 16) & 0xffu; }
__host__ __device__ inline unsigned ragged_count(unsigned e) { return e >> 24; }
int launch_frames_recur_ragged(const void* whh, const float* gi, const float* b_hn, const float* h0, float* hist, void* hr, float* h_state,
                               const RaggedMap& walk, int n, int rows, int n_t, int t, bool single_frame, int H, hipStream_t s,
                               bool f16 = false);
int launch_pool_commit_ragged(const PoolGeom& g, const int* slots, int n, const RaggedMap& rows, int n_rows, const float* h_ws,
                              const int* argmax, hipStream_t s);
```

### prego_amd/csrc/miniroad.cpp

```cpp
#include "miniroad_handle.h"

#include <algorithm>
#include <cstdarg>
#include <cstdio>
#include <cstdlib>

static thread_local std::string g_err;
static thread_local prego_miniroad* g_cur = nullptr;
HandleScope::HandleScope(prego_miniroad* h) { g_cur = h; }
HandleScope::~HandleScope() { g_cur = nullptr; }
int prego_fail_(int code, const char* fmt, ...) {
  char buf[512];
  va_list ap;
  va_start(ap, fmt);
  vsnprintf(buf, sizeof buf, fmt, ap);
  va_end(ap);
  g_err = buf;
  if (g_cur) g_cur->err = buf;
  return code;
}

const char* prego_tune_env(const char* name) {
#ifdef PREGO_DEBUG_ABI
  return getenv(name);
#else
  (void)name;
  return nullptr;
#endif
}

extern "C" const char* prego_miniroad_last_error(const prego_miniroad* h) { return h ? h->err.c_str() : "handle is NULL"; }

extern "C" int prego_abi_version(void) { return PREGO_ABI_VERSION; }
#ifdef PREGO_DEBUG_ABI
std::atomic<long long> g_dbg_mallocs{0}, g_dbg_syncs{0};
void launch_debug_hog(int xcd_lo, int kind, int ms, const void* buf, void* wbuf, size_t bytes, float* sink, hipStream_t s);
extern "C" int prego_debug_hog(int kind, int xcd_lo, int ms, const void* read_buf, void* write_buf, size_t bytes, float* sink, prego_stream_t stream) {
  if (kind < 1 || kind > 3 || xcd_lo < 0 || xcd_lo > 7 || ms <= 0 || !sink || ((kind & 2) && (!read_buf || !write_buf || bytes < (1u << 20))))
    return prego_fail_(PREGO_EINVAL, "debug hog: bad arguments");
  launch_debug_hog(xcd_lo, kind, ms, read_buf, write_buf, bytes, sink, (hipStream_t)stream);
  HIPCHK(hipGetLastError());
  return PREGO_OK;
}
extern "C" int prego_debug_alloc_count(int64_t* device_mallocs, int64_t* host_waits) {
  if (device_mallocs) *device_mallocs = g_dbg_mallocs.load();
  if (host_waits) *host_waits = g_dbg_syncs.load();
  return PREGO_OK;
}
#endif

extern "C" const char* prego_last_error(void) { return g_err.c_str(); }

extern "C" int prego_miniroad_create(prego_miniroad** out, int d_rgb, int d_flow, int emb, int hid, int n_classes,
                                     int compute_dtype) {
  return prego_miniroad_create_layers(out, d_rgb, d_flow, emb, hid, n_classes, 1, compute_dtype);
}
extern "C" int prego_miniroad_create_layers(prego_miniroad** out, int d_rgb, int d_flow, int emb, int hid, int n_classes, int num_layers,
                                            int compute_dtype) {
  if (!out) return prego_fail_(PREGO_EINVAL, "out is NULL");
  *out = nullptr;
  if (compute_dtype != PREGO_F32 && compute_dtype != PREGO_BF16 && compute_dtype != PREGO_F16 && compute_dtype != PREGO_F16X2)
    return prego_fail_(PREGO_EINVAL, "compute_dtype %d", compute_dtype);
  {
    const bool op16 = compute_dtype == PREGO_BF16 || compute_dtype == PREGO_F16;
    const bool ok = compute_dtype == PREGO_F16X2 ? hid == 1024 : gru_hidden_supported(op16, hid);
    if (!ok) return prego_fail_(PREGO_EINVAL, "hidden_dim %d unsupported with compute_dtype %d: 512 / 1024 / 2048 with 16-bit operands, 512 / 1024 with fp32 "
                                       "operands, 1024 with fp16x2 (the recurrence keeps its W_hh slice in registers)", hid, compute_dtype);
  }
  if (num_layers < 1 || num_layers > 2) return prego_fail_(PREGO_EINVAL, "num_layers %d: 1 or 2", num_layers);
  if (num_layers == 2 && compute_dtype == PREGO_F16X2)
    return prego_fail_(PREGO_EINVAL, "num_layers 2 with fp16x2 operands: the split-operand recurrence hands fp32 relu(h) to the classifier only (use fp32)");
  if (emb <= 0 || emb % 512 || emb > 4096) return prego_fail_(PREGO_EINVAL, "embedding_dim %d must be a multiple of 512, <= 4096", emb);
  if (d_rgb < 0 || d_flow < 0 || d_rgb + d_flow <= 0 || (d_rgb % 64) || (d_flow % 64))
    return prego_fail_(PREGO_EINVAL, "feature sizes %d/%d must be multiples of 64", d_rgb, d_flow);
  if (n_classes <= 0 || n_classes > 128) return prego_fail_(PREGO_EINVAL, "num_classes %d must be in 1..128", n_classes);
  int dev = 0;
  HIPCHK(hipGetDevice(&dev));
  hipDeviceProp_t prop;
  HIPCHK(hipGetDeviceProperties(&prop, dev));
  prego_miniroad* h = new prego_miniroad();
  h->d_rgb = d_rgb; h->d_flow = d_flow; h->emb = emb; h->hid = hid; h->ncls = n_classes;
  h->ncls_pad = (n_classes + 15) / 16 * 16;
  h->bf16 = compute_dtype == PREGO_BF16 || compute_dtype == PREGO_F16;
  h->f16 = compute_dtype == PREGO_F16;
  h->x2 = compute_dtype == PREGO_F16X2;
  h->n_cu = prop.multiProcessorCount;
  h->layers = num_layers;
  h->P = h->x2 ? hid / 16 : gru_group_size(h->bf16, hid);
  h->G = std::min(h->bf16 ? 8 : 4, h->n_cu / h->P);
  if (h->G < 1) { delete h; return prego_fail_(PREGO_EINVAL, "device has %d CUs, the recurrence needs >= %d", prop.multiProcessorCount, h->bf16 ? 32 : 64); }
  const size_t es = h->bf16 ? 2 : 4;
  const int din = d_rgb + d_flow, H = hid;
  hipError_t e = hipSuccess;
  auto A = [&](void** p, size_t bytes) { if (e == hipSuccess) e = hipMalloc(p, bytes); };
  A(&h->w1, (size_t)emb * din * es); A((void**)&h->b1, emb * 4); A((void**)&h->ln_g, emb * 4); A((void**)&h->ln_b, emb * 4);
  A(&h->w_ih, (size_t)3 * H * emb * es); A(&h->w_hh, (size_t)3 * H * H * es);
  A((void**)&h->bias2, 3 * H * 4); A((void**)&h->b_hn, H * 4);
  if (h->bf16 && H == 1024) { A(&h->w_ih_perm, (size_t)3 * H * emb * es); A((void**)&h->bias2_perm, 3 * H * 4); }
  A(&h->w_c, (size_t)h->ncls_pad * H * es); A((void**)&h->b_c, h->ncls_pad * 4);
  A(&h->hx, h->x2 ? gru_x2_hx_bytes(H, h->G) : gru_hx_bytes(h->bf16, H, h->G));
  if (h->x2) A((void**)&h->x2_scale, 6 * sizeof(float));
  A((void**)&h->flags, ((size_t)h->G * h->P + 16) * sizeof(unsigned));
  A((void**)&h->h_state, (size_t)num_layers * max_slots_of(h) * H * 4);
  if (num_layers == 2) {
    A(&h->l2_w_ih, (size_t)3 * H * H * es); A(&h->l2_w_hh, (size_t)3 * H * H * es);
    A((void**)&h->l2_bias2, 3 * H * 4); A((void**)&h->l2_b_hn, H * 4);
  }
  A((void**)&h->d_ptrs, (size_t)6 * max_clips_of(h) * sizeof(void*));
  h->cap_t = (size_t)131072 + 1;
  h->cap_c = (size_t)max_clips_of(h) + 64;
  A((void**)&h->d_rowoff, h->cap_t * 4); A((void**)&h->d_nact, h->cap_t * 4);
  A((void**)&h->d_sorted, h->cap_c * 4); A((void**)&h->d_seg_off, (h->cap_c + 1) * 4);
  A((void**)&h->d_seg_clip, h->cap_c * 4); A((void**)&h->d_seg_start, h->cap_c * 4);
  h->cap_b = (size_t)1 << 19;
  A((void**)&h->d_blkstep, h->cap_b * 4);
  h->pin_bytes = (size_t)6 * max_clips_of(h) * sizeof(void*) + 2 * h->cap_t * 4 + 4 * (h->cap_c + 1) * 4 + h->cap_b * 4 + 1024;
  if (e == hipSuccess) e = hipHostMalloc((void**)&h->pin, h->pin_bytes, hipHostMallocDefault);
  if (e == hipSuccess) e = hipEventCreateWithFlags(&h->pin_ev, hipEventDisableTiming);
  h->no_local = getenv("PREGO_GRU_NO_LOCAL") != nullptr;
  h->no_mt = getenv("PREGO_GRU_NO_MT") != nullptr;
  h->pack_prefetch = prego_tune_env("PREGO_NO_PACK_PREFETCH") == nullptr;
  h->prefetch_grid = 512;
  if (const char* pg = prego_tune_env("PREGO_PACK_PREFETCH_GRID")) h->prefetch_grid = atoi(pg);
  if (e == hipSuccess) {
    int lo = 0, hi = 0;
    static const bool plain = prego_tune_env("PREGO_SIDE_PRIO") != nullptr && atoi(prego_tune_env("PREGO_SIDE_PRIO")) == 0;
    if (!plain && hipDeviceGetStreamPriorityRange(&lo, &hi) == hipSuccess && lo != hi)
      e = hipStreamCreateWithPriority(&h->side, hipStreamNonBlocking, lo);
    else
      e = hipStreamCreateWithFlags(&h->side, hipStreamNonBlocking);
  }
  if (e == hipSuccess) e = hipEventCreateWithFlags(&h->ev_fork, hipEventDisableTiming);
  if (e == hipSuccess) e = hipEventCreateWithFlags(&h->ev_join, hipEventDisableTiming);
  A((void**)&h->stamps, 8 * sizeof(unsigned long long));
  A((void**)&h->tile_ctr, 4096 * sizeof(unsigned));
  if (e == hipSuccess) e = hipHostMalloc((void**)&h->pin_place, 64, hipHostMallocDefault);
  if (e == hipSuccess) e = hipEventCreateWithFlags(&h->ev_place, hipEventDisableTiming);
  if (e == hipSuccess) e = hipHostMalloc((void**)&h->pin_hs, 64, hipHostMallocDefault);
  if (e == hipSuccess) *(volatile unsigned*)h->pin_hs = 0u;
  if (e == hipSuccess) e = hipEventCreate(&h->chooser.ev_meas[0]);
  if (e == hipSuccess) e = hipEventCreate(&h->chooser.ev_meas[1]);
  h->xcd_overlap = getenv("PREGO_NO_XCD_OVERLAP") == nullptr;
  if (const char* sp = getenv("PREGO_SPLIT_PASS")) h->chooser.split_env = atoi(sp);
  A((void**)&h->st_scratch, (size_t)16 * ((size_t)emb * 6 + (size_t)3 * H * 8));
  if (e == hipSuccess) e = hipMemset(h->stamps, 0, 8 * sizeof(unsigned long long));
  h->use_stamps = prego_tune_env("PREGO_GRU_STAMPS") != nullptr;
  if (e == hipSuccess) e = hipMemset(h->hx, 0, h->x2 ? gru_x2_hx_bytes(H, h->G) : gru_hx_bytes(h->bf16, H, h->G));
  if (e == hipSuccess) e = hipMemset(h->flags, 0, ((size_t)h->G * h->P + 16) * sizeof(unsigned));
  if (e != hipSuccess) { prego_miniroad_destroy(h); return prego_fail_(PREGO_EHIP, "hipMalloc: %s", hipGetErrorString(e)); }
  h->abort_word = h->flags + (size_t)h->G * h->P;
  *out = h;
  return PREGO_OK;
}

#ifdef PREGO_DEBUG_ABI
#define PREGO_TEARDOWN(x) do { const hipError_t e_ = (x); if (e_ != hipSuccess) { fprintf(stderr, "prego_miniroad_destroy: %s -> %s\n", #x, hipGetErrorName(e_)); (void)hipGetLastError(); } } while (0)
#else
#define PREGO_TEARDOWN(x) do { if ((x) != hipSuccess) (void)hipGetLastError(); } while (0)
#endif
extern "C" void prego_miniroad_destroy(prego_miniroad* h) {
  if (!h) return;
  if (h->side) { PREGO_TEARDOWN(hipStreamSynchronize(h->side)); PREGO_TEARDOWN(hipStreamDestroy(h->side)); }
  void* ptrs[] = {h->w1, h->b1, h->ln_g, h->ln_b, h->w_ih, h->w_hh, h->bias2, h->b_hn, h->w_c, h->b_c, h->hx,
                  h->flags, h->h_state, h->stamps, h->tile_ctr, h->d_rowoff, h->d_nact, h->d_sorted, h->d_seg_off, h->d_seg_clip,
                  h->d_seg_start, h->d_ptrs, h->d_blkstep, h->st_scratch, h->x2_scale, h->l2_w_ih, h->l2_w_hh, h->l2_bias2, h->l2_b_hn, h->w_ih_perm, h->bias2_perm,
                  h->w_a, h->b_a, h->st_ant};
  for (size_t i = 0; i < sizeof ptrs / sizeof ptrs[0]; ++i)
    if (ptrs[i]) {
#ifdef PREGO_DEBUG_ABI
      const hipError_t e_ = hipFree(ptrs[i]);
      if (e_ != hipSuccess) { fprintf(stderr, "prego_miniroad_destroy: hipFree(ptrs[%zu] = %p) -> %s\n", i, ptrs[i], hipGetErrorName(e_)); (void)hipGetLastError(); }
#else
      PREGO_TEARDOWN(hipFree(ptrs[i]));
#endif
    }
  for (auto& ev : h->ev_pool) { PREGO_TEARDOWN(hipEventDestroy(ev.a)); PREGO_TEARDOWN(hipEventDestroy(ev.b)); }
  if (h->pin_ev) { if (h->pin_busy) PREGO_TEARDOWN(hipEventSynchronize(h->pin_ev)); PREGO_TEARDOWN(hipEventDestroy(h->pin_ev)); }
  if (h->pin) PREGO_TEARDOWN(hipHostFree(h->pin));
  if (h->ev_fork) PREGO_TEARDOWN(hipEventDestroy(h->ev_fork));
  if (h->ev_join) PREGO_TEARDOWN(hipEventDestroy(h->ev_join));
  if (h->ev_place) PREGO_TEARDOWN(hipEventDestroy(h->ev_place));
  for (hipEvent_t ev : h->chooser.ev_meas) if (ev) PREGO_TEARDOWN(hipEventDestroy(ev));
  for (hipEvent_t ev : h->ev_split) if (ev) PREGO_TEARDOWN(hipEventDestroy(ev));
  if (h->pin_place) PREGO_TEARDOWN(hipHostFree(h->pin_place));
  if (h->pin_hs) PREGO_TEARDOWN(hipHostFree(h->pin_hs));
  delete h;
}

extern "C" int prego_miniroad_max_clips(const prego_miniroad* h) { return h ? max_clips_of(h) : 0; }

extern "C" int prego_miniroad_set_weights(prego_miniroad* h, const float* layer1_w, const float* layer1_b,
                                          const float* ln_w, const float* ln_b, const float* w_ih, const float* w_hh,
                                          const float* b_ih, const float* b_hh, const float* fc_w, const float* fc_b,
                                          prego_stream_t stream) {
  HandleScope scope_(h);
  if (!h) return prego_fail_(PREGO_EINVAL, "handle is NULL");
  if (!layer1_w || !layer1_b || !ln_w || !ln_b || !w_ih || !w_hh || !b_ih || !b_hh || !fc_w || !fc_b)
    return prego_fail_(PREGO_EINVAL, "set_weights: NULL tensor");
  hipStream_t s = (hipStream_t)stream;
  const int din = h->d_rgb + h->d_flow, E = h->emb, H = h->hid;
  if (h->x2) {
    launch_x2_weight_split(layer1_w, E, din, h->w1, h->x2_scale + 0, s);
    launch_x2_weight_split(w_ih, 3 * H, E, h->w_ih, h->x2_scale + 2, s);
    launch_x2_weight_split(w_hh, 3 * H, H, h->w_hh, h->x2_scale + 4, s);
  } else {
    launch_pad_convert(h->bf16, layer1_w, E, din, din, h->w1, E, din, s, h->f16);
    launch_pad_convert(h->bf16, w_ih, 3 * H, E, E, h->w_ih, 3 * H, E, s, h->f16);
    launch_pad_convert(h->bf16, w_hh, 3 * H, H, H, h->w_hh, 3 * H, H, s, h->f16);
  }
  launch_pad_convert(h->bf16, fc_w, h->ncls, H, H, h->w_c, h->ncls_pad, H, s, h->f16);
  launch_pad_convert(false, fc_b, 1, h->ncls, h->ncls, h->b_c, 1, h->ncls_pad, s);
  HIPCHK(hipMemcpyAsync(h->b1, layer1_b, E * 4, hipMemcpyDeviceToDevice, s));
  HIPCHK(hipMemcpyAsync(h->ln_g, ln_w, E * 4, hipMemcpyDeviceToDevice, s));
  HIPCHK(hipMemcpyAsync(h->ln_b, ln_b, E * 4, hipMemcpyDeviceToDevice, s));
  launch_add_vec(b_ih, b_hh, h->bias2, 3 * H, 2 * H, s);
  h->perm_stale = true;
  HIPCHK(hipMemcpyAsync(h->b_hn, b_hh + 2 * H, H * 4, hipMemcpyDeviceToDevice, s));
  HIPCHK(hipGetLastError());
  h->have_weights = true;
  return PREGO_OK;
}

extern "C" int prego_miniroad_set_gru_layer(prego_miniroad* h, int layer, const float* w_ih, const float* w_hh, const float* b_ih,
                                            const float* b_hh, prego_stream_t stream) {
  HandleScope scope_(h);
  if (!h) return prego_fail_(PREGO_EINVAL, "handle is NULL");
  if (layer != 1 || h->layers != 2) return prego_fail_(PREGO_EINVAL, "set_gru_layer: layer %d of a %d-layer handle (layer 0 comes with set_weights)", layer, h->layers);
  if (!w_ih || !w_hh || !b_ih || !b_hh) return prego_fail_(PREGO_EINVAL, "set_gru_layer: NULL tensor");
  hipStream_t s = (hipStream_t)stream;
  const int H = h->hid;
  launch_pad_convert(h->bf16, w_ih, 3 * H, H, H, h->l2_w_ih, 3 * H, H, s, h->f16);
  launch_pad_convert(h->bf16, w_hh, 3 * H, H, H, h->l2_w_hh, 3 * H, H, s, h->f16);
  launch_add_vec(b_ih, b_hh, h->l2_bias2, 3 * H, 2 * H, s);
  HIPCHK(hipMemcpyAsync(h->l2_b_hn, b_hh + 2 * H, H * 4, hipMemcpyDeviceToDevice, s));
  HIPCHK(hipGetLastError());
  h->have_layer2 = true;
  return PREGO_OK;
}

extern "C" int prego_miniroad_set_anticipation(prego_miniroad* h, int ant_len, const float* w_a, const float* b_a, prego_stream_t stream) {
  HandleScope scope_(h);
  if (!h) return prego_fail_(PREGO_EINVAL, "handle is NULL");
  if (h->x2) return prego_fail_(PREGO_EINVAL, "set_anticipation: fp16x2 (split-operand) handles have no anticipation head; use fp32, bf16 or fp16");
  if (h->layers != 1)
    return prego_fail_(PREGO_EINVAL, "set_anticipation: num_layers %d - MiniROADA runs one GRU layer (its h0 is (1, B, H), rnn.py:122)", h->layers);
  if (ant_len < 1 || ant_len > 32) return prego_fail_(PREGO_EINVAL, "set_anticipation: anticipation_length %d must be in 1..32", ant_len);
  if (!w_a || !b_a) return prego_fail_(PREGO_EINVAL, "set_anticipation: NULL tensor");
  hipStream_t s = (hipStream_t)stream;
  const int H = h->hid;
  const size_t es = h->bf16 ? 2 : 4, need = (size_t)ant_len * H * H * es;
  if (need > h->w_a_cap || ant_len > h->ant_len) {
    HIPCHK(hipStreamSynchronize(s));
    if (h->w_a) { HIPCHK(hipFree(h->w_a)); h->w_a = nullptr; }
    if (h->b_a) { HIPCHK(hipFree(h->b_a)); h->b_a = nullptr; }
    if (h->st_ant) { HIPCHK(hipFree(h->st_ant)); h->st_ant = nullptr; }
    h->w_a_cap = 0;
    HIPCHK(hipMalloc(&h->w_a, need));
    HIPCHK(hipMalloc((void**)&h->b_a, (size_t)ant_len * H * 4));
    if (h->bf16 && H == 1024) HIPCHK(hipMalloc(&h->st_ant, (size_t)16 * ant_len * H * 2));
    h->w_a_cap = need;
  }
  launch_pad_convert(h->bf16, w_a, ant_len * H, H, H, h->w_a, ant_len * H, H, s, h->f16);
  HIPCHK(hipMemcpyAsync(h->b_a, b_a, (size_t)ant_len * H * 4, hipMemcpyDeviceToDevice, s));
  HIPCHK(hipGetLastError());
  h->ant_len = ant_len;
  return PREGO_OK;
}

extern "C" int prego_miniroad_set_resident(prego_miniroad* h, void* device_buffer, size_t bytes) {
  HandleScope scope_(h);
  if (!h) return prego_fail_(PREGO_EINVAL, "handle is NULL");
  if ((device_buffer == nullptr) != (bytes == 0)) return prego_fail_(PREGO_EINVAL, "set_resident: buffer %p with %zu bytes", device_buffer, bytes);
  if ((uintptr_t)device_buffer & 255) return prego_fail_(PREGO_EINVAL, "set_resident: the buffer must be 256-byte aligned");
  h->res_buf = (char*)device_buffer; h->res_bytes = bytes;
  return PREGO_OK;
}

void launch_guard_publish(const unsigned* abort_word, float* dst, hipStream_t s);
extern "C" int prego_miniroad_guard_publish(prego_miniroad* h, float* dst, prego_stream_t stream) {
  HandleScope scope_(h);
  if (!h || !dst) return prego_fail_(PREGO_EINVAL, "guard_publish: NULL argument");
  launch_guard_publish(h->abort_word, dst, (hipStream_t)stream);
  HIPCHK(hipGetLastError());
  return PREGO_OK;
}
extern "C" int prego_miniroad_set_peer_guard(prego_miniroad* h, const float* reduced_word) {
  HandleScope scope_(h);
  if (!h) return prego_fail_(PREGO_EINVAL, "handle is NULL");
  h->peer_guard = reduced_word;
  return PREGO_OK;
}

EventPair* ev_begin(prego_miniroad* h, int kind, hipStream_t s) {
  if (!h->timing) return nullptr;
  if (h->ev_used == h->ev_pool.size()) {
    EventPair p;
    if (hipEventCreate(&p.a) != hipSuccess || hipEventCreate(&p.b) != hipSuccess) return nullptr;
    h->ev_pool.push_back(p);
    h->ev_kind.push_back(kind);
  }
  h->ev_kind[h->ev_used] = kind;
  EventPair* p = &h->ev_pool[h->ev_used++];
  (void)hipEventRecord(p->a, s);
  return p;
}
void ev_end(EventPair* p, hipStream_t s) { if (p) (void)hipEventRecord(p->b, s); }

extern "C" int prego_miniroad_check(prego_miniroad* h, prego_stream_t stream) {
  HandleScope scope_(h);
  if (!h) return prego_fail_(PREGO_EINVAL, "handle is NULL");
  HIPCHK(hipStreamSynchronize((hipStream_t)stream));
  unsigned ab = 0;
  HIPCHK(hipMemcpy(&ab, h->abort_word, sizeof ab, hipMemcpyDeviceToHost));
  if (ab) {
    (void)hipMemset(h->abort_word, 0, sizeof ab);
    if (ab == 0x200u)
      return prego_fail_(PREGO_ETIMEOUT, "data-parallel training: a recurrence / BPTT kernel of ANOTHER rank timed out; every rank skipped the optimizer "
                  "steps from that one on (weights unchanged since the last good step) [code 0x200]");
    if (ab >= 2) {
      h->chooser.split_env = 0;
      return prego_fail_(PREGO_ETIMEOUT, "split pass: a wait timed out behind a successful start handshake [code 0x%x]; the results of that call are "
                  "invalid, this handle now uses the chunked pass (PREGO_SPLIT_PASS=0 selects it from the start)", ab);
    }
    return prego_fail_(PREGO_ETIMEOUT, "GRU recurrence kernel timed out waiting for a producer workgroup (not all %d workgroups resident?) [code 0x%x]",
                h->G * h->P, ab);
  }
  return PREGO_OK;
}

extern "C" int prego_miniroad_timing_enable(prego_miniroad* h, int enable) {
  if (!h) return prego_fail_(PREGO_EINVAL, "handle is NULL");
  h->timing = enable != 0;
  h->ev_used = 0;
  h->gemm_flop = 0;
  h->pack_bytes = 0;
  return PREGO_OK;
}

extern "C" int prego_miniroad_timing_read(prego_miniroad* h, double* gemm_ms, int64_t* gemm_launches, double* gemm_flop,
                                          double* gru_ms, int64_t* gru_launches, double* pack_ms,
                                          int64_t* pack_launches, double* pack_bytes) {
  HandleScope scope_(h);
  if (!h) return prego_fail_(PREGO_EINVAL, "handle is NULL");
  double ms[5] = {0, 0, 0, 0, 0};
  int64_t n[5] = {0, 0, 0, 0, 0};
  for (size_t i = 0; i < h->ev_used; ++i) {
    HIPCHK(hipEventSynchronize(h->ev_pool[i].b));
    float t = 0;
    HIPCHK(hipEventElapsedTime(&t, h->ev_pool[i].a, h->ev_pool[i].b));
    ms[h->ev_kind[i]] += t;
    n[h->ev_kind[i]]++;
  }
  if (gemm_ms) *gemm_ms = ms[0];
  if (gemm_launches) *gemm_launches = n[0];
  if (gemm_flop) *gemm_flop = h->gemm_flop;
  if (gru_ms) *gru_ms = ms[1];
  if (gru_launches) *gru_launches = n[1];
  if (pack_ms) *pack_ms = ms[2];
  if (pack_launches) *pack_launches = n[2];
  if (pack_bytes) *pack_bytes = h->pack_bytes;
  h->ev_used = 0;
  h->gemm_flop = 0;
  h->pack_bytes = 0;
  return PREGO_OK;
}

extern "C" int prego_miniroad_pass_info(const prego_miniroad* h, int32_t* mode, int32_t* n_steps, int32_t* n_slots) {
  if (!h) return prego_fail_(PREGO_EINVAL, "handle is NULL");
  if (mode) *mode = h->split_r;
  if (n_steps) *n_steps = h->t_max;
  if (n_slots) *n_slots = h->n_slots;
  return PREGO_OK;
}

#ifdef PREGO_DEBUG_ABI
extern "C" int prego_miniroad_debug_stamps(prego_miniroad* h, unsigned long long* out8) {
  if (!h || !out8) return prego_fail_(PREGO_EINVAL, "NULL");
  HIPCHK(hipDeviceSynchronize());
  HIPCHK(hipMemcpy(out8, h->stamps, 8 * sizeof(unsigned long long), hipMemcpyDeviceToHost));
  HIPCHK(hipMemset(h->stamps, 0, 8 * sizeof(unsigned long long)));
  return PREGO_OK;
}

extern "C" int prego_debug_set_abort(prego_miniroad* h, unsigned value, prego_stream_t stream) {
  if (!h) return prego_fail_(PREGO_EINVAL, "handle is NULL");
  HIPCHK(hipMemsetD32Async((hipDeviceptr_t)h->abort_word, (int)value, 1, (hipStream_t)stream));
  return PREGO_OK;
}
#endif
```

### prego_amd/csrc/miniroad_handle.h

```cpp
#pragma once
#include "host_common.h"

#include <cstdarg>
#include <cstdint>
#include <cstdio>
#include <string>
#include <vector>
#ifdef PREGO_DEBUG_ABI
#include <atomic>
#endif

#ifdef PREGO_DEBUG_ABI
extern __attribute__((visibility("hidden"))) std::atomic<long long> g_dbg_mallocs, g_dbg_syncs;
#define hipMalloc(p, n) (++g_dbg_mallocs, (hipMalloc)(p, n))
#define hipStreamSynchronize(s) (++g_dbg_syncs, (hipStreamSynchronize)(s))
#define hipEventSynchronize(e) (++g_dbg_syncs, (hipEventSynchronize)(e))
#endif

struct EventPair { hipEvent_t a, b; };

struct prego_miniroad {
  int d_rgb, d_flow, emb, hid, ncls, ncls_pad;
  bool bf16;
  bool f16 = false;
  bool x2 = false;
  float* x2_scale = nullptr;
  int n_cu;
  int G, P;
  void* w1 = nullptr;
  float* b1 = nullptr;
  float* ln_g = nullptr;
  float* ln_b = nullptr;
  void* w_ih = nullptr;
  void* w_hh = nullptr;
  float* bias2 = nullptr;
  void* w_ih_perm = nullptr; float* bias2_perm = nullptr; bool perm_stale = true;
  float* b_hn = nullptr;
  void* w_c = nullptr;
  float* b_c = nullptr;
  bool have_weights = false;
  int ant_len = 0; void* w_a = nullptr; float* b_a = nullptr; size_t w_a_cap = 0;
  void* st_ant = nullptr;
  bool ant_kept = false; bool ant_grads_set = false;
  std::vector<const float*> ant_d; float* ant_g_w = nullptr; float* ant_g_b = nullptr;
  int layers = 1;
  void* l2_w_ih = nullptr; void* l2_w_hh = nullptr; float* l2_bias2 = nullptr; float* l2_b_hn = nullptr; bool have_layer2 = false;
  void* hx = nullptr;
  unsigned* flags = nullptr;
  unsigned* abort_word = nullptr;
  float* h_state = nullptr;
  unsigned long long* stamps = nullptr;
  char* st_scratch = nullptr;
  bool use_stamps = false;
  float drop_p = 0.f;
  unsigned long long drop_seed = 0;
  int kept_kx = 0;
  int kept_rows = 0;
  float* g_l2[4] = {nullptr, nullptr, nullptr, nullptr};
  hipEvent_t bwd_ev[2] = {nullptr, nullptr};
  prego_bucket_fn bwd_cb = nullptr; void* bwd_cb_user = nullptr;
  std::vector<int32_t> plan_lens;
  std::vector<int> h_rowoff, h_nact, h_sorted;
  std::vector<int> h_seg_off, h_seg_clip, h_seg_start;
  std::vector<int> h_blkstep;
  int* d_blkstep = nullptr; size_t cap_b = 0;
  int n_slots = 0;
  bool plan_single = true;
  bool plan_want_single = false;
  int plan_host_row_bytes = 0;
  std::vector<int> feed_upto; std::vector<hipEvent_t> feed_ev; size_t feed_pos = 0; int feed_row_bytes = 0;
  int t_max = 0;
  int* d_rowoff = nullptr; int* d_nact = nullptr; int* d_sorted = nullptr;
  int* d_seg_off = nullptr; int* d_seg_clip = nullptr; int* d_seg_start = nullptr;
  size_t cap_t = 0, cap_c = 0;
  void** d_ptrs = nullptr;
  char* pin = nullptr; size_t pin_bytes = 0; hipEvent_t pin_ev = nullptr; bool pin_busy = false;
  bool plan_dirty = false;
  bool no_local = false;
  bool no_mt = false;
  hipStream_t side = nullptr; hipEvent_t ev_fork = nullptr, ev_join = nullptr; bool pack_prefetch = true;
  unsigned* tile_ctr = nullptr; bool xcd_overlap = false;
  int placement = -1; unsigned* pin_place = nullptr; hipEvent_t ev_place = nullptr; bool place_pending = false;
  int prefetch_grid = 0;
  int split_r = 0; int plan_force_slots = 0;
  double plan_cost_us = 0;
  struct Chooser {
    int split_env = -1;
    std::vector<int32_t> split_seen_lens; int split_seen_key = -1, split_seen_r = 3; double split_seen_est_c = 0, split_seen_est_s = 0;
    hipEvent_t ev_meas[2] = {nullptr, nullptr}; bool meas_pending = false, meas_armed = false; int meas_mode = 0; double meas_est = 0;
    double ratio_chunked = 1.0, ratio_split = 1.0; bool have_ratio_chunked = false, have_ratio_split = false, split_warm = false;
    int split_fails = 0; long long split_skip = 0; long long split_fallbacks = 0;
  } chooser;
  char* res_buf = nullptr; size_t res_bytes = 0;
  const float* peer_guard = nullptr;
  unsigned* pin_hs = nullptr; unsigned hs_seq = 0;
  int dbg_fault = 0;
  hipEvent_t ev_split[4] = {nullptr, nullptr, nullptr, nullptr};
  double split_rec_ms = 0, split_ff_ms = 0; long long split_passes = 0, split_steps = 0; bool split_ev_pending = false;
  std::string err;
  bool timing = false;
  std::vector<EventPair> ev_pool;
  std::vector<int> ev_kind;
  size_t ev_used = 0;
  double gemm_flop = 0, pack_bytes = 0;
};

#pragma GCC visibility push(hidden)

struct HandleScope {
  explicit HandleScope(prego_miniroad* h);
  ~HandleScope();
};

static inline int max_slots_of(const prego_miniroad* h) { return h->G * 16 * (h->x2 ? 2 : gru_max_tiles()); }
#define PREGO_MAX_CLIPS 8192
static inline int max_clips_of(const prego_miniroad*) { return PREGO_MAX_CLIPS; }

EventPair* ev_begin(prego_miniroad* h, int kind, hipStream_t s);
void ev_end(EventPair* p, hipStream_t s);

int build_plan(prego_miniroad* h, int n, const int32_t* lens, bool want_single, int host_row_bytes = 0, int slots_arg = 0);
SlotPlan device_plan(const prego_miniroad* h);
int stage_tables(prego_miniroad* h, const void* const* tab4, size_t tab_count, hipStream_t s);

struct RowBytes { size_t x, y, e, gi, hr, hraw, gates, stats, map, l2keep, total; };
bool inter16(const prego_miniroad* h, int flags);
RowBytes row_bytes(const prego_miniroad* h, bool with_flow, int flags);
struct FwdLayout {
  RowBytes rb;
  long long cap_rows;
  size_t X, Y, E, GI, HR, HRAW, KR, KZ, KN, KG, STATS, HR0, HRAW2, KR2, KZ2, KN2, KG2, RM;
  size_t total;
  void* at(void* workspace, size_t off) const { return off ? (char*)workspace + off : nullptr; }
};
FwdLayout fwd_layout(const prego_miniroad* h, bool with_flow, int flags, size_t workspace_bytes);
long long fwd_rows_fit(const RowBytes& rb, size_t workspace_bytes);
size_t fwd_bytes_for_rows(const RowBytes& rb, long long rows);

struct SplitRings { size_t x, y, e, gi, total; int ring_units; };
SplitRings split_rings(const prego_miniroad* h, int R);
bool split_workspace_ok(const prego_miniroad* h, int R, size_t workspace_bytes);
size_t split_buf_need(const prego_miniroad* h, long long total);
bool split_resident_ok(const prego_miniroad* h, long long total);

struct AntOut {
  bool call = false;
  float* const* out = nullptr;
  int32_t* const* arg = nullptr;
  bool wanted() const { return call && (out || arg); }
};
struct FwdTables { const float* const* rgb; const float* const* flow; float* const* out; int* const* arg; };
int forward_split(prego_miniroad* h, const AntOut& ao, int R, int flags, bool with_flow, bool in16, int kx, const SlotPlan& plan,
                  const FwdTables& tb, void* workspace, size_t workspace_bytes, hipStream_t s, bool* fell_back);

int ant_head(prego_miniroad* h, const AntOut& ao, const void* HR, const SlotPlan& plan, int row0, int nrows, int flags, hipStream_t s);

int step_refusals(prego_miniroad* h, int n_streams, int n_max, const float* rgb, const float* flow, const float* h_state, bool ant);

struct RaggedPlan { RaggedMap by_stream, walk; int alive[32]; int kmax, rows; };
int ragged_plan(const char* who, int n, const int32_t* n_frames, RaggedPlan* p);

struct WsCarver {
  size_t o = 0;
  size_t take(size_t bytes) { const size_t at = o; o += align_up(bytes, 256); return at; }
};
__attribute__((format(printf, 6, 7))) static inline int workspace_refusal(const char* who, const char* hint, void* ws, size_t bytes, size_t need,
                                                                          const char* what, ...) {
  if (!ws || bytes < need) {
    char buf[96];
    va_list ap;
    va_start(ap, what);
    vsnprintf(buf, sizeof buf, what, ap);
    va_end(ap);
    return prego_fail_(PREGO_EINVAL, "%s: workspace %p with %zu bytes, %s need %zu (%s)", who, ws, bytes, buf, need, hint);
  }
  if ((uintptr_t)ws & 255) return prego_fail_(PREGO_EINVAL, "%s: the workspace must be 256-byte aligned", who);
  return 0;
}

#pragma GCC visibility pop
```

### prego_amd/csrc/miniroad_split.cpp

```cpp
#include "miniroad_handle.h"

#include <algorithm>
#include <chrono>
#include <cstdlib>
#include <mutex>
#include <thread>

static int tuned_pow2(const char* name, int dflt) {
  const char* v = prego_tune_env(name);
  const int x = v ? atoi(v) : 0;
  return (x >= 16 && (x & (x - 1)) == 0) ? x : dflt;
}
static int split_gi_ring_units(int R) { return tuned_pow2("PREGO_SPLIT_GI_RING", R <= 3 ? 32 : 256); }
static const int kSplitRingPerXcd = (prego_tune_env("PREGO_SPLIT_RING_PER_XCD") && atoi(prego_tune_env("PREGO_SPLIT_RING_PER_XCD")) >= 12 &&
                                     atoi(prego_tune_env("PREGO_SPLIT_RING_PER_XCD")) % 4 == 0) ? atoi(prego_tune_env("PREGO_SPLIT_RING_PER_XCD")) : 24;
static const int kSplitSg = (prego_tune_env("PREGO_SPLIT_SG") && kSplitRingPerXcd % std::max(1, atoi(prego_tune_env("PREGO_SPLIT_SG"))) == 0)
                                ? std::max(1, atoi(prego_tune_env("PREGO_SPLIT_SG"))) : 2;
static int split_chunk_shift(int R) { return prego_tune_env("PREGO_SPLIT_CHUNK_SHIFT") ? atoi(prego_tune_env("PREGO_SPLIT_CHUNK_SHIFT")) : (R <= 3 ? 3 : 6); }
SplitRings split_rings(const prego_miniroad* h, int R) {
  SplitRings g;
  g.ring_units = kSplitRingPerXcd * (8 - R);
  g.x = align_up((size_t)g.ring_units * 256 * (size_t)(h->d_rgb + h->d_flow) * 2, 256);
  g.y = align_up((size_t)g.ring_units * 256 * (size_t)h->emb * 2, 256);
  g.e = g.y;
  g.gi = align_up((size_t)split_gi_ring_units(R) * 256 * (size_t)3 * h->hid * 2, 256);
  g.total = g.x + g.y + g.e + g.gi;
  return g;
}
bool split_workspace_ok(const prego_miniroad* h, int R, size_t workspace_bytes) { return workspace_bytes >= split_rings(h, R).total; }

size_t split_buf_need(const prego_miniroad* h, long long total) {
  const long long n_units = (total + 255) / 256;
  const int shift = split_chunk_shift(1);
  const long long n_chunks = (n_units + (1 << shift) - 1) >> shift;
  return align_up((size_t)total * h->hid * 2, 256) + align_up((size_t)total * 8, 256) + align_up(((size_t)4 * n_units + 2 * (size_t)n_chunks + 32) * 4, 256);
}
bool split_resident_ok(const prego_miniroad* h, long long total) { return h->res_buf && split_buf_need(h, total) <= h->res_bytes; }

extern "C" size_t prego_miniroad_resident_bytes(const prego_miniroad* h, int n_clips, const int32_t* lens, int flags) {
  if (!h || n_clips <= 0 || !lens) return 0;
  if ((flags & PREGO_FWD_KEEP) || h->layers != 1) return 0;
  long long total = 0;
  for (int i = 0; i < n_clips; ++i) total += lens[i] > 0 ? lens[i] : 0;
  if (total < 65536) return 0;
  const RowBytes rb = row_bytes(h, true, flags);
  size_t need = align_up((size_t)total * rb.hr, 256);
  if (h->bf16 && h->hid == 1024) need = std::max(need, split_buf_need(h, total));
  return need <= ((size_t)24 << 30) + ((size_t)1 << 30) ? need : 0;
}

static std::mutex g_split_mu;
static hipEvent_t g_split_last[64] = {};

int forward_split(prego_miniroad* h, const AntOut& ao, int R, int flags, bool with_flow, bool in16, int kx, const SlotPlan& plan,
                  const FwdTables& tb, void* workspace, size_t workspace_bytes, hipStream_t s, bool* fell_back) {
  *fell_back = false;
  const int H = h->hid, E = h->emb, din = h->d_rgb + h->d_flow;
  const int total = h->h_rowoff[h->t_max];
  const int n_units = (total + 255) / 256;
  const int chunk_shift = split_chunk_shift(R), gi_ring = split_gi_ring_units(R);
  const int upc = 1 << chunk_shift;
  const int n_chunks = (n_units + upc - 1) >> chunk_shift;
  const SplitRings rg = split_rings(h, R);
  if (workspace_bytes < rg.total) return prego_fail_(PREGO_EWORKSPACE, "split pass: workspace %zu B < %zu B of rings", workspace_bytes, rg.total);
  char* wp = (char*)workspace;
  unsigned short* X = (unsigned short*)wp; wp += rg.x;
  unsigned short* Y = (unsigned short*)wp; wp += rg.y;
  unsigned short* Eb = (unsigned short*)wp; wp += rg.e;
  unsigned short* GI = (unsigned short*)wp;
  const size_t hr_bytes = align_up((size_t)total * H * 2, 256), rm_bytes = align_up((size_t)total * 8, 256);
  const size_t n_ctr = (size_t)4 * n_units + 2 * (size_t)n_chunks + 32;
  if (!h->chooser.split_warm) { h->chooser.meas_armed = false; h->chooser.split_warm = true; }
  if (!split_resident_ok(h, total)) return prego_fail_(PREGO_EWORKSPACE, "split pass: resident buffer %zu B < %zu B", h->res_bytes, split_buf_need(h, total));
  char* HR = h->res_buf;
  char* RM = HR + hr_bytes;
  unsigned* ctr = (unsigned*)(RM + rm_bytes);
  unsigned* tick = ctr; unsigned* hs_word = ctr + 8; unsigned* ff_here = ctr + 16; unsigned* pack_done = ctr + 32; unsigned* l1_cnt = pack_done + n_units; unsigned* ln_done = l1_cnt + n_units;
  unsigned* wih_cnt = ln_done + n_units; unsigned* gi_cnt = wih_cnt + n_units; unsigned* rec_cnt = gi_cnt + n_chunks;
  HIPCHK(hipMemsetAsync(ctr, 0, n_ctr * 4, s));
  HIPCHK(hipMemsetAsync(h->h_state, 0, (size_t)h->n_slots * H * 4, s));
  PassHandshake hs{};
  h->hs_seq = (h->hs_seq + 1u) & 0x3FFFFFFFu;
  if (h->hs_seq == 0u) h->hs_seq = 1u;
  hs.word = hs_word; hs.ff_here = ff_here; hs.host = h->pin_hs; hs.seq = h->hs_seq; hs.ticks_lead = 5000000u; hs.ticks_all = 10000000u;
  int fault = 0;
#ifdef PREGO_DEBUG_ABI
  fault = h->dbg_fault; h->dbg_fault = 0;
  if (fault == 3 || fault == 4) {
    HIPCHK(hipMemsetD32Async((hipDeviceptr_t)hs_word, PREGO_HS_GO, 1, s));
    HIPCHK(hipMemsetD32Async((hipDeviceptr_t)ff_here, 1, 8, s));
    if (fault == 3) HIPCHK(hipMemsetD32Async((hipDeviceptr_t)rec_cnt, R * h->P * 4, n_chunks, s));
    else HIPCHK(hipMemsetD32Async((hipDeviceptr_t)gi_cnt, upc, n_chunks, s));
    hs.host = nullptr;
  }
#endif

  FfPassArgs fa{};
  fa.rgb_ptrs = tb.rgb; fa.flow_ptrs = with_flow ? tb.flow : nullptr; fa.plan = plan; fa.rowmap = RM;
  fa.d_rgb = h->d_rgb; fa.d_flow = with_flow ? h->d_flow : 0; fa.in16 = in16 ? 1 : 0; fa.kx = kx;
  fa.w1 = (const unsigned short*)h->w1; fa.ld_w1 = din; fa.b1 = h->b1; fa.ln_g = h->ln_g; fa.ln_b = h->ln_b; fa.ln_eps = 1e-5f;
  fa.w_ih = (const unsigned short*)h->w_ih_perm; fa.bias2 = h->bias2_perm; fa.E = E; fa.n3 = 3 * H;
  fa.X = X; fa.Y = Y; fa.Eb = Eb; fa.GI = GI; fa.ring_units = rg.ring_units; fa.gi_ring_units = gi_ring;
  fa.total_rows = total; fa.n_units = n_units; fa.xcd_lo = R; fa.chunk_unit_shift = chunk_shift;
  fa.rec_expect = R * h->P * 4; fa.nt1 = E / 256; fa.nt2 = 3 * H / 256;
  static const int lag1 = prego_tune_env("PREGO_SPLIT_LAG1") ? atoi(prego_tune_env("PREGO_SPLIT_LAG1")) : 2;
  static const int lag2 = prego_tune_env("PREGO_SPLIT_LAG2") ? atoi(prego_tune_env("PREGO_SPLIT_LAG2")) : 3;
  static const int lag3 = prego_tune_env("PREGO_SPLIT_LAG3") ? atoi(prego_tune_env("PREGO_SPLIT_LAG3")) : 4;
  static const bool want_stats = prego_tune_env("PREGO_SPLIT_STATS") != nullptr;
  fa.sg = kSplitSg; fa.lag1 = lag1; fa.lag2 = lag2; fa.lag3 = lag3; fa.f16 = h->f16 ? 1 : 0;
  static const int ff_cus = prego_tune_env("PREGO_SPLIT_FF_CUS") ? atoi(prego_tune_env("PREGO_SPLIT_FF_CUS")) : 0;
  fa.max_wg = ff_cus;
  fa.stats = want_stats ? h->stamps : nullptr;
#ifdef PREGO_DEBUG_ABI
  static const int dbg = prego_tune_env("PREGO_SPLIT_DBG") ? atoi(prego_tune_env("PREGO_SPLIT_DBG")) : 0;
  fa.dbg = dbg;
#endif
  fa.tick = tick; fa.pack_done = pack_done; fa.l1_cnt = l1_cnt; fa.ln_done = ln_done; fa.wih_cnt = wih_cnt; fa.gi_cnt = gi_cnt;
  fa.rec_cnt = rec_cnt; fa.abort_word = h->abort_word; fa.hs = hs;
  const int ring_sr = kSplitRingPerXcd / kSplitSg;
  if (lag1 < 1 || lag2 <= lag1 || lag3 <= lag2 || lag1 >= ring_sr || lag2 - ring_sr >= lag1 || lag3 - ring_sr >= lag2)
    return prego_fail_(PREGO_EINVAL, "split pass: lags %d %d %d", lag1, lag2, lag3);

  GruArgs ga{};
  ga.whh = h->w_hh; ga.b_hn = h->b_hn; ga.gi = GI; ga.gi_bf16 = 1; ga.f16 = h->f16 ? 1 : 0; ga.h_relu_out = HR; ga.h_raw_out = nullptr;
  ga.h_state = h->h_state; ga.hx = h->hx; ga.flags = h->flags; ga.abort_word = h->abort_word;
  ga.rowoff = h->d_rowoff; ga.nact = h->d_nact; ga.t0 = 0; ga.t1 = h->t_max; ga.row_base = 0; ga.rows = 0;
  ga.n_clips = h->n_slots; ga.G = h->G; ga.seg_off = h->plan_single ? nullptr : h->d_seg_off;
  ga.seg_start = h->plan_single ? nullptr : h->d_seg_start; ga.stamps = (h->use_stamps && !want_stats) ? h->stamps : nullptr;
  ga.sync = h->flags; ga.armed = 0; ga.Gd = R;
  ga.gi_cnt = gi_cnt; ga.rec_cnt = rec_cnt; ga.chunk_shift = chunk_shift + 8; ga.n_chunks = n_chunks;
  ga.units_per_chunk = upc; ga.units_last = n_units - upc * (n_chunks - 1); ga.gi_row_mask = (unsigned)gi_ring * 256u - 1u;
  ga.hs = hs;

  struct SideJoin {
    prego_miniroad* h; bool pending = false;
    ~SideJoin() { if (pending) (void)hipStreamSynchronize(h->side); }
  } side_join{h};
  launch_gru_arm(true, H, h->G, h->hx, h->flags, s);
  if (h->perm_stale) {
    launch_permute_gi_rows(h->w_ih, h->bias2, h->w_ih_perm, h->bias2_perm, H, E, s);
    h->perm_stale = false;
  }
  std::lock_guard<std::mutex> split_lock(g_split_mu);
  int dev_ = 0;
  HIPCHK(hipGetDevice(&dev_));
  const bool dev_ok = dev_ >= 0 && dev_ < 64;
  if (dev_ok && g_split_last[dev_]) HIPCHK(hipStreamWaitEvent(s, g_split_last[dev_], 0));
  HIPCHK(hipEventRecord(h->ev_fork, s));
  HIPCHK(hipStreamWaitEvent(h->side, h->ev_fork, 0));
  const bool run_ff = fault != 2 && fault != 4, run_rec = fault != 1 && fault != 3;
  const size_t ev_mark = h->ev_used;
  EventPair* evf = run_ff ? ev_begin(h, 2, h->side) : nullptr;
  if (run_ff && launch_ff_pass(fa, h->side)) return prego_fail_(PREGO_EINVAL, "split pass: feed-forward shape E=%d kx=%d", E, kx);
  ev_end(evf, h->side);
  side_join.pending = true;
  HIPCHK(hipEventRecord(h->ev_join, h->side));
  EventPair* evr = run_rec ? ev_begin(h, 1, s) : nullptr;
  if (run_rec && launch_gru_recurrence_pass(H, ga, s)) return prego_fail_(PREGO_EINVAL, "split pass: recurrence launch");
  ev_end(evr, s);
  HIPCHK(hipStreamWaitEvent(s, h->ev_join, 0));
  side_join.pending = false;
  if (dev_ok) {
    if (!g_split_last[dev_]) HIPCHK(hipEventCreateWithFlags(&g_split_last[dev_], hipEventDisableTiming));
    HIPCHK(hipEventRecord(g_split_last[dev_], s));
  }
  if (fault == 3 || fault == 4) { HIPCHK(hipGetLastError()); return PREGO_OK; }
  {
    const std::chrono::steady_clock::time_point t0 = std::chrono::steady_clock::now();
    unsigned state = 0u; long long polls = 0;
    for (;;) {
      const unsigned v = __atomic_load_n(h->pin_hs, __ATOMIC_ACQUIRE);
      if ((v >> 2) == hs.seq && (v & 3u)) { state = v & 3u; break; }
      if ((++polls & 63) == 0) {
        if (hipStreamQuery(s) == hipSuccess) {
          const unsigned v2 = __atomic_load_n(h->pin_hs, __ATOMIC_ACQUIRE);
          state = ((v2 >> 2) == hs.seq && (v2 & 3u)) ? (v2 & 3u) : PREGO_HS_FAIL;
          break;
        }
        if (std::chrono::steady_clock::now() - t0 > std::chrono::seconds(300))
          return prego_fail_(PREGO_ETIMEOUT, "split pass: the stream did not reach the pass within 300 s");
      }
      std::this_thread::sleep_for(std::chrono::microseconds(20));
    }
    if (state != PREGO_HS_GO) {
      h->ev_used = ev_mark;
      h->chooser.meas_armed = false;
      *fell_back = true;
      HIPCHK(hipGetLastError());
      return PREGO_OK;
    }
  }
  if (h->timing) { h->gemm_flop += 2.0 * total * ((double)E * kx + 3.0 * H * E); h->split_passes++; h->split_steps += h->t_max; }
  if ((tb.out || tb.arg) &&
      launch_head_softmax(true, HR, h->w_c, h->b_c, plan, 0, total, H, h->ncls, (flags & PREGO_FWD_SOFTMAX) ? 1 : 0, tb.out, tb.arg, s,
                          RM, h->f16))
    return prego_fail_(PREGO_EINVAL, "head: unsupported num_classes %d", h->ncls);
  if (int rc_a = ant_head(h, ao, HR, plan, 0, total, flags, s)) return rc_a;
  if (h->chooser.meas_armed) { HIPCHK(hipEventRecord(h->chooser.ev_meas[1], s)); h->chooser.meas_pending = true; h->chooser.meas_armed = false; }
  HIPCHK(hipGetLastError());
  return PREGO_OK;
}

#ifdef PREGO_DEBUG_ABI
extern "C" int prego_debug_split_fault(prego_miniroad* h, int mode) {
  if (!h || mode < 0 || mode > 4) return prego_fail_(PREGO_EINVAL, "debug split fault: mode %d", mode);
  h->dbg_fault = mode;
  return PREGO_OK;
}
#endif
```

Before: 25.02 million frames/s.

## Add lookahead ticket claiming and prologue prefetch to split feed-forward pass

Restructures the persistent feed-forward worker so that, while finishing the current tile, a workgroup claims its next ticket, probes the dependency counters (including via buffer-load-to-LDS), and pre-stages the next GEMM tile's first K-slices into shared memory when it is ready. Ticket decoding and dependency rules move into a shared header so the host can test them. This is meant to hide the claim, poll and pipeline-fill latency between consecutive tiles. In exchange it makes the worker loop and synchronisation more complex, and a wrong readiness check could read stale data or cause hangs. Lookahead is on by default, and the debug build gains hooks to toggle it and read per-phase stats.

```diff
diff --git a/include/prego_amd_debug.h b/include/prego_amd_debug.h
--- a/include/prego_amd_debug.h
+++ b/include/prego_amd_debug.h
@@ -15,6 +15,10 @@
                             unsigned* counter, int grid, prego_stream_t stream);
 
 int prego_debug_split_fault(prego_miniroad* h, int mode);
+int prego_debug_split_lookahead(prego_miniroad* h, int on);
+int prego_debug_split_stats(prego_miniroad* h, unsigned long long* out10);
+int prego_debug_ff_ticket(int k, int n_units, int nf, int q, int sg, int nt1, int nt2, int lag1, int lag2, int lag3, int ring_units,
+                          int gi_ring_units, int chunk_unit_shift, int32_t* out16);
 int prego_debug_split_state(const prego_miniroad* h, int64_t* fallbacks, int32_t* fails, int64_t* skip, int32_t* split_env);
 int prego_debug_set_abort(prego_miniroad* h, unsigned value, prego_stream_t stream);
 int prego_debug_alloc_count(int64_t* device_mallocs, int64_t* host_waits);
diff --git a/prego_amd/_lib.py b/prego_amd/_lib.py
--- a/prego_amd/_lib.py
+++ b/prego_amd/_lib.py
@@ -45,7 +45,8 @@
 DEBUG_SYMBOLS = ["prego_miniroad_debug_stamps", "prego_debug_gemm_bf16", "prego_debug_attention_bwd", "prego_debug_attention_fwd",
                  "prego_debug_recurrence_only", "prego_debug_gemm_worker", "prego_debug_head_only",
                  "prego_debug_split_fault", "prego_debug_split_state", "prego_debug_set_abort", "prego_debug_alloc_count", "prego_debug_hog",
-                 "prego_debug_ant_full_span", "prego_debug_gemm_tn", "prego_debug_gemm_nt"]
+                 "prego_debug_ant_full_span", "prego_debug_gemm_tn", "prego_debug_gemm_nt",
+                 "prego_debug_split_lookahead", "prego_debug_split_stats", "prego_debug_ff_ticket"]
 
 
 class PregoError(RuntimeError):
@@ -198,6 +199,9 @@
         lib.prego_debug_gemm_tn.argtypes = [i32, i32, vp, i32, vp, i32, vp, vp, vp, i32, i32, i32, i32, i32, vp, vp]
         lib.prego_debug_gemm_nt.argtypes = [i32, i32, vp, i32, vp, i32, vp, vp, i32, i32, i32, i32, vp]
         lib.prego_debug_split_fault.argtypes = [vp, i32]
+        lib.prego_debug_split_lookahead.argtypes = [vp, i32]
+        lib.prego_debug_split_stats.argtypes = [vp, C.POINTER(C.c_uint64)]
+        lib.prego_debug_ff_ticket.argtypes = [i32] * 13 + [C.POINTER(C.c_int32)]
         lib.prego_debug_split_state.argtypes = [vp, C.POINTER(i64), C.POINTER(i32), C.POINTER(i64), C.POINTER(i32)]
         lib.prego_debug_set_abort.argtypes = [vp, C.c_uint32, vp]
         lib.prego_debug_alloc_count.argtypes = [C.POINTER(i64), C.POINTER(i64)]
diff --git a/prego_amd/csrc/ff_pass.hip b/prego_amd/csrc/ff_pass.hip
--- a/prego_amd/csrc/ff_pass.hip
+++ b/prego_amd/csrc/ff_pass.hip
@@ -1,6 +1,7 @@
 #include "common.h"
 #include "kernels.h"
 #include "pass_handshake.h"
+#include "ff_ticket.h"
 
 #define FBK 64
 #define FHALF 16384
@@ -27,146 +28,373 @@
   }
 }
 
-template <typename OT, bool SC1OUT>
-__device__ __forceinline__ void ffp_tile(char* smem, const bf16_t* __restrict__ A, int lda, int rows, const bf16_t* __restrict__ B, int ldb,
-                                         const float* __restrict__ bias, bf16_t* __restrict__ C, int ldc, int K) {
+enum { NX_STATE = 0, NX_TYPE = 1, NX_UNIT = 2, NX_NB = 3, NX_READY = 4, NX_SEEN = 6, NX_WORDS = 8 };
+enum { NX_JOB = 1, NX_END = 2 };
+
+__device__ __forceinline__ FfGeom ffp_geom(const FfPassArgs& a) { return FfGeom{a.sg, a.nt1, a.nt2, a.lag1, a.lag2, a.lag3}; }
+__device__ __forceinline__ int ffp_queue(const FfPassArgs& a) {
+  return (int)(__builtin_amdgcn_s_getreg((3 << 11) | 20) & 7) - a.xcd_lo;
+}
+__device__ __forceinline__ unsigned ffp_lane_id() { return __builtin_amdgcn_mbcnt_hi(~0u, __builtin_amdgcn_mbcnt_lo(~0u, 0u)); }
+__device__ __forceinline__ const unsigned* ffp_counter(const FfPassArgs& a, const FfWait& w) {
+  const unsigned* c0 = a.pack_done; const unsigned* c1 = a.l1_cnt; const unsigned* c2 = a.ln_done; const unsigned* c3 = a.wih_cnt;
+  const unsigned* c4 = a.rec_cnt;
+  const unsigned* p = w.counter == FF_CNT_PACK ? c0 : w.counter == FF_CNT_L1 ? c1 : w.counter == FF_CNT_LN ? c2 : w.counter == FF_CNT_WIH ? c3 : c4;
+  return p + w.index;
+}
+__device__ __forceinline__ unsigned ffp_need(const FfPassArgs& a, const FfWait& w) {
+  const unsigned all = (unsigned)a.rec_expect;
+  return w.counter == FF_CNT_REC ? all : (unsigned)w.need;
+}
+__device__ __forceinline__ bool ffp_job_wait(const FfPassArgs& a, int type, int u, int which, FfWait& w) {
+  return ff_job_wait(type, u, ffp_geom(a), a.ring_units, a.gi_ring_units, a.chunk_unit_shift, which, w);
+}
+
+__device__ __forceinline__ void ffp_claim_finish(const FfPassArgs& a, unsigned k, int* s_nx) {
+  const int q = ffp_queue(a), nf = 8 - a.xcd_lo;
+  const FfGeom g = ffp_geom(a);
+  const int n_q = ff_queue_units(a.n_units, q, nf), n_rounds = ff_queue_rounds(n_q, g);
+  for (;;) {
+    const FfJob b = ff_ticket_decode((int)k, g);
+    if (b.round >= n_rounds) { s_nx[NX_STATE] = NX_END; s_nx[NX_READY] = 0; return; }
+    if (b.i >= 0 && b.i < n_q) {
+      s_nx[NX_TYPE] = b.type; s_nx[NX_UNIT] = q + b.i * nf; s_nx[NX_NB] = b.nb; s_nx[NX_READY] = 0; s_nx[NX_STATE] = NX_JOB;
+      return;
+    }
+    k = __hip_atomic_fetch_add(a.tick + q, 1u, __ATOMIC_RELAXED, __HIP_MEMORY_SCOPE_AGENT);
+  }
+}
+__device__ __forceinline__ void ffp_claim(const FfPassArgs& a, int* s_nx) {
+  ffp_claim_finish(a, __hip_atomic_fetch_add(a.tick + ffp_queue(a), 1u, __ATOMIC_RELAXED, __HIP_MEMORY_SCOPE_AGENT), s_nx);
+}
+
+__device__ __forceinline__ unsigned ffp_probe_issue(const FfPassArgs& a, int* s_nx, unsigned ln) {
+  if (s_nx[NX_STATE] != NX_JOB) return 0u;
+  FfWait w;
+  if (!ffp_job_wait(a, s_nx[NX_TYPE], s_nx[NX_UNIT], (int)ln, w)) return 0u;
+  return __hip_atomic_load(ffp_counter(a, w), __ATOMIC_RELAXED, __HIP_MEMORY_SCOPE_AGENT);
+}
+__device__ __forceinline__ void ffp_probe_eval(const FfPassArgs& a, int* s_nx, unsigned ln, unsigned seen) {
+  bool ok = s_nx[NX_STATE] == NX_JOB;
+  if (ok) {
+    FfWait w;
+    if (ffp_job_wait(a, s_nx[NX_TYPE], s_nx[NX_UNIT], (int)ln, w)) ok = seen >= ffp_need(a, w);
+  }
+  const unsigned long long all = __builtin_amdgcn_ballot_w64(ok);
+  if (ln == 0) s_nx[NX_READY] = (all & 3ull) == 3ull ? 1 : 0;
+}
+__device__ __forceinline__ void ffp_probe_dma(const FfPassArgs& a, int* s_nx) {
+  if (__builtin_amdgcn_readfirstlane(s_nx[NX_STATE]) != NX_JOB) return;
+  const int type = __builtin_amdgcn_readfirstlane(s_nx[NX_TYPE]), u = __builtin_amdgcn_readfirstlane(s_nx[NX_UNIT]);
+  const bool lane0 = ffp_lane_id() == 0;
+#pragma unroll
+  for (int which = 0; which < 2; ++which) {
+    FfWait w;
+    if (!ffp_job_wait(a, type, u, which, w)) continue;
+    const unsigned long long pa = (unsigned long long)ffp_counter(a, w);
+    const unsigned long long pu = ((unsigned long long)(unsigned)__builtin_amdgcn_readfirstlane((int)(unsigned)(pa >> 32)) << 32) |
+                                  (unsigned)__builtin_amdgcn_readfirstlane((int)(unsigned)pa);
+    const __amdgpu_buffer_rsrc_t rs = __builtin_amdgcn_make_buffer_rsrc((void*)pu, 0, 4, 0x00020000);
+    if (lane0) __builtin_amdgcn_raw_ptr_buffer_load_lds(rs, (__attribute__((address_space(3))) void*)(s_nx + NX_SEEN + which), 4, 0, 0, 0, AUX_SC1);
+  }
+}
+__device__ __forceinline__ void ffp_probe_dma_eval(const FfPassArgs& a, int* s_nx, unsigned ln) {
+  bool ok = s_nx[NX_STATE] == NX_JOB;
+  if (ok) {
+    FfWait w;
+    if (ffp_job_wait(a, s_nx[NX_TYPE], s_nx[NX_UNIT], (int)ln, w)) ok = (unsigned)s_nx[NX_SEEN + (ln & 1)] >= ffp_need(a, w);
+  }
+  const unsigned long long all = __builtin_amdgcn_ballot_w64(ok);
+  if (ln == 0) s_nx[NX_READY] = (all & 3ull) == 3ull ? 1 : 0;
+}
+__device__ __forceinline__ void ffp_probe(const FfPassArgs& a, int* s_nx) {
+  const unsigned ln = ffp_lane_id();
+  if (ln < 2) ffp_probe_eval(a, s_nx, ln, ffp_probe_issue(a, s_nx, ln));
+}
+
+__device__ __forceinline__ void ffp_bar_lds() {
+  __builtin_amdgcn_sched_barrier(0);
+  asm volatile("s_waitcnt lgkmcnt(0)\n\ts_barrier" ::: "memory");
+  __builtin_amdgcn_sched_barrier(0);
+}
+
+struct FfTile {
+  const bf16_t* A; const bf16_t* B; const float* bias; bf16_t* C;
+  int lda, ldb, ldc, K, rows;
+  bool sc1;
+};
+__device__ __forceinline__ FfTile ffp_tile_desc(const FfPassArgs& a, int type, int u, int nb) {
+  const bf16_t* X = a.X; const bf16_t* Eb = a.Eb; const bf16_t* w1 = a.w1; const bf16_t* w_ih = a.w_ih; const float* b1 = a.b1; const float* bias2 = a.bias2;
+  bf16_t* Y = a.Y; bf16_t* GI = a.GI;
+  const int kx = a.kx, E = a.E, ld_w1 = a.ld_w1, n3 = a.n3;
+  const bool l1 = type == FF_JOB_L1;
+  FfTile t;
+  const int row0 = u * 256;
+  t.rows = a.total_rows - row0 < 256 ? a.total_rows - row0 : 256;
+  const size_t slot = (size_t)(u % a.ring_units) * 256, gslot = (size_t)(u & (a.gi_ring_units - 1)) * 256;
+  t.lda = l1 ? kx : E; t.ldb = l1 ? ld_w1 : E; t.ldc = l1 ? E : n3; t.K = t.lda; t.sc1 = !l1;
+  t.A = (l1 ? X : Eb) + slot * t.lda;
+  t.B = (l1 ? w1 : w_ih) + (size_t)nb * 256 * t.ldb;
+  t.bias = (l1 ? b1 : bias2) + nb * 256;
+  t.C = (l1 ? Y + slot * E : GI + gslot * n3) + nb * 256;
+  return t;
+}
+
+__device__ __forceinline__ void ffp_stage_prologue(char* smem, const FfTile& t) {
   int tid = threadIdx.x;
   asm volatile("" : "+v"(tid));
   const int lane = tid & 63;
   const int wave = __builtin_amdgcn_readfirstlane(tid >> 6);
-  const int grp = wave >> 2, wc = wave & 3;
-  const int nk = K / FBK;
   const int sr = lane >> 3, scp = lane & 7;
   int a_off[2], b_off[2];
 #pragma unroll
   for (int i = 0; i < 2; ++i) {
     const int r = (wave * 2 + i) * 8 + sr;
-    a_off[i] = r * lda * 2 + ((scp ^ ((r >> 1) & 7)) << 4);
-    b_off[i] = r * ldb * 2 + ((scp ^ ffp_key_b(r)) << 4);
-  }
-  const __amdgpu_buffer_rsrc_t rs_a = __builtin_amdgcn_make_buffer_rsrc((void*)A, 0, rows * lda * 2, 0x00020000);
-  const __amdgpu_buffer_rsrc_t rs_b = __builtin_amdgcn_make_buffer_rsrc((void*)B, 0, 256 * ldb * 2, 0x00020000);
+    a_off[i] = r * t.lda * 2 + ((scp ^ ((r >> 1) & 7)) << 4);
+    b_off[i] = r * t.ldb * 2 + ((scp ^ ffp_key_b(r)) << 4);
+  }
+  const __amdgpu_buffer_rsrc_t rs_a = __builtin_amdgcn_make_buffer_rsrc((void*)t.A, 0, t.rows * t.lda * 2, 0x00020000);
+  const __amdgpu_buffer_rsrc_t rs_b = __builtin_amdgcn_make_buffer_rsrc((void*)t.B, 0, 256 * t.ldb * 2, 0x00020000);
   auto stage_a = [&](int hf, int kt) {
     char* dst = smem + (kt & 1) * FBUF + hf * FHALF + wave * 2048;
-    const int so = hf * 128 * lda * 2 + kt * (FBK * 2);
+    const int so = hf * 128 * t.lda * 2 + kt * (FBK * 2);
 #pragma unroll
     for (int i = 0; i < 2; ++i)
       __builtin_amdgcn_raw_ptr_buffer_load_lds(rs_a, (__attribute__((address_space(3))) void*)(dst + i * 1024), 16, a_off[i], so, 0, 0);
   };
   auto stage_b = [&](int hf, int kt) {
     char* dst = smem + (kt & 1) * FBUF + (2 + hf) * FHALF + wave * 2048;
-    const int so = hf * 128 * ldb * 2 + kt * (FBK * 2);
+    const int so = hf * 128 * t.ldb * 2 + kt * (FBK * 2);
 #pragma unroll
     for (int i = 0; i < 2; ++i)
       __builtin_amdgcn_raw_ptr_buffer_load_lds(rs_b, (__attribute__((address_space(3))) void*)(dst + i * 1024), 16, b_off[i], so, 0, 0);
   };
-  const int fr = lane & 15, fq = lane >> 4;
-  bf16x8 a0[2][4], a1[2][4], b0[2][2], b1[2][2];
-  auto read_a = [&](bf16x8 (&af)[2][4], int slot, int kt) {
-    const char* base = smem + (kt & 1) * FBUF + slot * FHALF;
-#pragma unroll
-    for (int ks = 0; ks < 2; ++ks)
-#pragma unroll
-      for (int i = 0; i < 4; ++i) {
-        const int r = grp * 64 + i * 16 + fr;
-        af[ks][i] = *(const bf16x8*)(base + r * 128 + (((ks * 4 + fq) ^ ((r >> 1) & 7)) << 4));
-      }
-  };
-  auto read_b = [&](bf16x8 (&bf)[2][2], int slot, int kt) {
-    const char* base = smem + (kt & 1) * FBUF + slot * FHALF;
-#pragma unroll
-    for (int ks = 0; ks < 2; ++ks)
-#pragma unroll
-      for (int j = 0; j < 2; ++j) {
-        const int r = wc * 32 + (fr >> 2) * 8 + j * 4 + (fr & 3);
-        bf[ks][j] = *(const bf16x8*)(base + r * 128 + (((ks * 4 + fq) ^ ffp_key_b(r)) << 4));
-      }
-  };
-  f32x4 acc[2][2][4][2];
-#pragma unroll
-  for (int x = 0; x < 2; ++x)
-#pragma unroll
-    for (int y = 0; y < 2; ++y)
-#pragma unroll
-      for (int i = 0; i < 4; ++i)
-#pragma unroll
-        for (int j = 0; j < 2; ++j) acc[x][y][i][j] = (f32x4){0.f, 0.f, 0.f, 0.f};
-  auto mma = [&](f32x4 (&c)[4][2], const bf16x8 (&af)[2][4], const bf16x8 (&bf)[2][2]) {
-    asm volatile("s_waitcnt lgkmcnt(0)" ::: "memory");
-    __builtin_amdgcn_sched_barrier(0);
-    __builtin_amdgcn_s_setprio(1);
-#pragma unroll
-    for (int ks = 0; ks < 2; ++ks)
-#pragma unroll
-      for (int i = 0; i < 4; ++i)
-#pragma unroll
-        for (int j = 0; j < 2; ++j) c[i][j] = op16<OT>::mfma(bf[ks][j], af[ks][i], c[i][j]);
-    __builtin_amdgcn_s_setprio(0);
-    __builtin_amdgcn_sched_barrier(0);
-  };
-  auto bar = [&]() {
-    __builtin_amdgcn_sched_barrier(0);
-    __builtin_amdgcn_s_barrier();
-    __builtin_amdgcn_sched_barrier(0);
-  };
   stage_a(0, 0); stage_b(0, 0); stage_b(1, 0); stage_a(1, 0);
   stage_a(0, 1); stage_b(0, 1); stage_b(1, 1);
-  FF_WAIT(10);
-  bar();
-  read_a(a0, 0, 0);
-  if (grp == 1) bar();
-  for (int kt = 0; kt < nk; ++kt) {
-    const bool full = kt + 2 < nk;
-    read_b(b0, 2, kt);
-    if (kt + 1 < nk) stage_a(1, kt + 1);
-    if (full) FF_WAIT(10); else FF_WAIT(0);
+}
+
+enum { FST_LAST = 8, FST_T0 = 9, FST_C0 = 10, FST_TILE_END = 11, FST_BETWEEN = 12, FST_BETWEEN_N = 13, FST_WORDS = 14 };
+__device__ __forceinline__ void ffp_stat(unsigned long long* s_stat, int slot) {
+  const unsigned long long n = __builtin_amdgcn_s_memrealtime();
+  s_stat[slot] += n - s_stat[FST_LAST];
+  s_stat[FST_LAST] = n;
+}
+
+template <typename OT>
+__device__ __forceinline__ void ffp_tiles(char* smem, const FfPassArgs& a, int* s_nx, unsigned long long* s_stat, int type, int u, int nb,
+                                          bool pre, const bool look) {
+  bool pub = false, p_wih = false;
+  int p_u = 0;
+  for (;;) {
+    type = __builtin_amdgcn_readfirstlane(type); u = __builtin_amdgcn_readfirstlane(u); nb = __builtin_amdgcn_readfirstlane(nb);
+    const FfTile t = ffp_tile_desc(a, type, u, nb);
+    int tid = threadIdx.x;
+    asm volatile("" : "+v"(tid));
+    const int lane = tid & 63;
+    const int wave = __builtin_amdgcn_readfirstlane(tid >> 6);
+    const bool stats = a.stats != nullptr;
+    const int grp = wave >> 2, wc = wave & 3;
+    const int nk = t.K / FBK;
+    const int kp = nk > 2 ? nk - 2 : 1;
+    const int sr = lane >> 3, scp = lane & 7;
+    int a_off[2], b_off[2];
+#pragma unroll
+    for (int i = 0; i < 2; ++i) {
+      const int r = (wave * 2 + i) * 8 + sr;
+      a_off[i] = r * t.lda * 2 + ((scp ^ ((r >> 1) & 7)) << 4);
+      b_off[i] = r * t.ldb * 2 + ((scp ^ ffp_key_b(r)) << 4);
+    }
+    const __amdgpu_buffer_rsrc_t rs_a = __builtin_amdgcn_make_buffer_rsrc((void*)t.A, 0, t.rows * t.lda * 2, 0x00020000);
+    const __amdgpu_buffer_rsrc_t rs_b = __builtin_amdgcn_make_buffer_rsrc((void*)t.B, 0, 256 * t.ldb * 2, 0x00020000);
+    auto stage_a = [&](int hf, int kt) {
+      char* dst = smem + (kt & 1) * FBUF + hf * FHALF + wave * 2048;
+      const int so = hf * 128 * t.lda * 2 + kt * (FBK * 2);
+#pragma unroll
+      for (int i = 0; i < 2; ++i)
+        __builtin_amdgcn_raw_ptr_buffer_load_lds(rs_a, (__attribute__((address_space(3))) void*)(dst + i * 1024), 16, a_off[i], so, 0, 0);
+    };
+    auto stage_b = [&](int hf, int kt) {
+      char* dst = smem + (kt & 1) * FBUF + (2 + hf) * FHALF + wave * 2048;
+      const int so = hf * 128 * t.ldb * 2 + kt * (FBK * 2);
+#pragma unroll
+      for (int i = 0; i < 2; ++i)
+        __builtin_amdgcn_raw_ptr_buffer_load_lds(rs_b, (__attribute__((address_space(3))) void*)(dst + i * 1024), 16, b_off[i], so, 0, 0);
+    };
+    const int fr = lane & 15, fq = lane >> 4;
+    bf16x8 a0[2][4], a1[2][4], b0[2][2], b1[2][2];
+    auto read_a = [&](bf16x8 (&af)[2][4], int slot, int kt) {
+      const char* base = smem + (kt & 1) * FBUF + slot * FHALF;
+#pragma unroll
+      for (int ks = 0; ks < 2; ++ks)
+#pragma unroll
+        for (int i = 0; i < 4; ++i) {
+          const int r = grp * 64 + i * 16 + fr;
+          af[ks][i] = *(const bf16x8*)(base + r * 128 + (((ks * 4 + fq) ^ ((r >> 1) & 7)) << 4));
+        }
+    };
+    auto read_b = [&](bf16x8 (&bf)[2][2], int slot, int kt) {
+      const char* base = smem + (kt & 1) * FBUF + slot * FHALF;
+#pragma unroll
+      for (int ks = 0; ks < 2; ++ks)
+#pragma unroll
+        for (int j = 0; j < 2; ++j) {
+          const int r = wc * 32 + (fr >> 2) * 8 + j * 4 + (fr & 3);
+          bf[ks][j] = *(const bf16x8*)(base + r * 128 + (((ks * 4 + fq) ^ ffp_key_b(r)) << 4));
+        }
+    };
+    f32x4 acc[2][2][4][2];
+#pragma unroll
+    for (int x = 0; x < 2; ++x)
+#pragma unroll
+      for (int y = 0; y < 2; ++y)
+#pragma unroll
+        for (int i = 0; i < 4; ++i)
+#pragma unroll
+          for (int j = 0; j < 2; ++j) acc[x][y][i][j] = (f32x4){0.f, 0.f, 0.f, 0.f};
+    auto mma = [&](f32x4 (&c)[4][2], const bf16x8 (&af)[2][4], const bf16x8 (&bf)[2][2]) {
+      asm volatile("s_waitcnt lgkmcnt(0)" ::: "memory");
+      __builtin_amdgcn_sched_barrier(0);
+      __builtin_amdgcn_s_setprio(1);
+#pragma unroll
+      for (int ks = 0; ks < 2; ++ks)
+#pragma unroll
+        for (int i = 0; i < 4; ++i)
+#pragma unroll
+          for (int j = 0; j < 2; ++j) c[i][j] = op16<OT>::mfma(bf[ks][j], af[ks][i], c[i][j]);
+      __builtin_amdgcn_s_setprio(0);
+      __builtin_amdgcn_sched_barrier(0);
+    };
+    auto bar = [&]() {
+      __builtin_amdgcn_sched_barrier(0);
+      __builtin_amdgcn_s_barrier();
+      __builtin_amdgcn_sched_barrier(0);
+    };
+    if (!pre) {
+      stage_a(0, 0); stage_b(0, 0); stage_b(1, 0); stage_a(1, 0);
+      stage_a(0, 1); stage_b(0, 1); stage_b(1, 1);
+    }
+    FF_WAIT(10);
     bar();
-    mma(acc[0][0], a0, b0);
-    bar();
-    read_b(b1, 3, kt);
-    if (full) { stage_a(0, kt + 2); FF_WAIT(10); } else FF_WAIT(0);
-    bar();
-    mma(acc[0][1], a0, b1);
-    bar();
-    read_a(a1, 1, kt);
-    if (full) { stage_b(0, kt + 2); FF_WAIT(10); } else FF_WAIT(0);
-    bar();
-    mma(acc[1][1], a1, b1);
-    bar();
-    if (kt + 1 < nk) read_a(a0, 0, kt + 1);
-    if (full) { stage_b(1, kt + 2); FF_WAIT(10); } else FF_WAIT(0);
-    bar();
-    mma(acc[1][0], a1, b0);
-    bar();
-  }
-  if (grp == 0) bar();
-  float4 bv[2][2];
-#pragma unroll
-  for (int y = 0; y < 2; ++y)
-#pragma unroll
-    for (int j = 0; j < 2; ++j) bv[y][j] = *(const float4*)(bias + y * 128 + wc * 32 + fq * 8 + j * 4);
-  const __amdgpu_buffer_rsrc_t rs_c = __builtin_amdgcn_make_buffer_rsrc((void*)C, 0, rows * ldc * 2, 0x00020000);
-#pragma unroll
-  for (int x = 0; x < 2; ++x)
-#pragma unroll
-    for (int y = 0; y < 2; ++y) {
-      const int n = y * 128 + wc * 32 + fq * 8;
-#pragma unroll
-      for (int i = 0; i < 4; ++i) {
-        const int m = x * 128 + grp * 64 + i * 16 + fr;
-        const f32x4 v0 = acc[x][y][i][0], v1 = acc[x][y][i][1];
-        u32x4 pk;
-        pk[0] = op16<OT>::pack2_sat(v0[0] + bv[y][0].x, v0[1] + bv[y][0].y); pk[1] = op16<OT>::pack2_sat(v0[2] + bv[y][0].z, v0[3] + bv[y][0].w);
-        pk[2] = op16<OT>::pack2_sat(v1[0] + bv[y][1].x, v1[1] + bv[y][1].y); pk[3] = op16<OT>::pack2_sat(v1[2] + bv[y][1].z, v1[3] + bv[y][1].w);
-        if constexpr (SC1OUT) __builtin_amdgcn_raw_buffer_store_b128(pk, rs_c, (m * ldc + n) * 2, 0, AUX_SC1);
-        else __builtin_amdgcn_raw_buffer_store_b128(pk, rs_c, (m * ldc + n) * 2, 0, 0);
-      }
-    }
-}
-
-template <typename OT, bool IN16>
+    if (stats && wave == 0 && ffp_lane_id() == 0 && s_stat[FST_TILE_END]) {
+      s_stat[FST_BETWEEN] += __builtin_amdgcn_s_memrealtime() - s_stat[FST_TILE_END];
+      s_stat[FST_BETWEEN_N] += 1;
+    }
+    read_a(a0, 0, 0);
+    if (grp == 1) bar();
+    for (int kt = 0; kt < nk; ++kt) {
+      const bool full = kt + 2 < nk;
+      const bool hook0 = look && wave == 0 && kt == 0;
+      unsigned got = 0u;
+      if (hook0) {
+        const unsigned ln = ffp_lane_id();
+        if (ln < (pub ? 2u : 1u)) {
+          unsigned* p = ln == 0 ? a.tick + ffp_queue(a) : (p_wih ? a.wih_cnt : a.l1_cnt) + p_u;
+          got = __hip_atomic_fetch_add(p, 1u, __ATOMIC_RELAXED, __HIP_MEMORY_SCOPE_AGENT);
+        }
+      }
+      if (look && wave == 0 && kt == kp) ffp_probe_dma(a, s_nx);
+      read_b(b0, 2, kt);
+      if (kt + 1 < nk) stage_a(1, kt + 1);
+      if (full) FF_WAIT(10); else FF_WAIT(0);
+      bar();
+      mma(acc[0][0], a0, b0);
+      bar();
+      read_b(b1, 3, kt);
+      if (full) { stage_a(0, kt + 2); FF_WAIT(10); } else FF_WAIT(0);
+      bar();
+      mma(acc[0][1], a0, b1);
+      bar();
+      if (hook0) {
+        const unsigned ln = ffp_lane_id();
+        if (ln == 0) ffp_claim_finish(a, got, s_nx);
+        else if (ln == 1 && pub && p_wih && got + 1u == (unsigned)a.nt2)
+          __hip_atomic_fetch_add(a.gi_cnt + (p_u >> a.chunk_unit_shift), 1u, __ATOMIC_RELAXED, __HIP_MEMORY_SCOPE_AGENT);
+      }
+      read_a(a1, 1, kt);
+      if (full) { stage_b(0, kt + 2); FF_WAIT(10); } else FF_WAIT(0);
+      bar();
+      mma(acc[1][1], a1, b1);
+      bar();
+      if (kt + 1 < nk) read_a(a0, 0, kt + 1);
+      if (full) { stage_b(1, kt + 2); FF_WAIT(10); } else FF_WAIT(0);
+      bar();
+      mma(acc[1][0], a1, b0);
+      bar();
+    }
+    if (grp == 0) bar();
+    if (stats && wave == 0 && ffp_lane_id() == 0) s_stat[FST_TILE_END] = __builtin_amdgcn_s_memrealtime();
+    bool chain = false;
+    int n_type = 0, n_u = 0, n_nb = 0;
+    if (look) {
+      if (wave == 0) {
+        const unsigned ln = ffp_lane_id();
+        if (ln < 2) ffp_probe_dma_eval(a, s_nx, ln);
+      }
+      ffp_bar_lds();
+      n_type = __builtin_amdgcn_readfirstlane(s_nx[NX_TYPE]); n_u = __builtin_amdgcn_readfirstlane(s_nx[NX_UNIT]);
+      n_nb = __builtin_amdgcn_readfirstlane(s_nx[NX_NB]);
+      chain = __builtin_amdgcn_readfirstlane(s_nx[NX_STATE]) == NX_JOB && __builtin_amdgcn_readfirstlane(s_nx[NX_READY]) != 0 &&
+              (n_type == FF_JOB_L1 || n_type == FF_JOB_WIH);
+    }
+    int tid_e = threadIdx.x;
+    asm volatile("" : "+v"(tid_e));
+    const int efr = tid_e & 15, efq = (tid_e & 63) >> 4;
+    float4 bv[2][2];
+#pragma unroll
+    for (int y = 0; y < 2; ++y)
+#pragma unroll
+      for (int j = 0; j < 2; ++j) bv[y][j] = *(const float4*)(t.bias + y * 128 + wc * 32 + efq * 8 + j * 4);
+    auto epilogue = [&]() __attribute__((always_inline)) {
+      const __amdgpu_buffer_rsrc_t rs_c = __builtin_amdgcn_make_buffer_rsrc((void*)t.C, 0, t.rows * t.ldc * 2, 0x00020000);
+  #pragma unroll
+      for (int x = 0; x < 2; ++x)
+  #pragma unroll
+        for (int y = 0; y < 2; ++y) {
+          const int n = y * 128 + wc * 32 + efq * 8;
+  #pragma unroll
+          for (int i = 0; i < 4; ++i) {
+            const int m = x * 128 + grp * 64 + i * 16 + efr;
+            const f32x4 v0 = acc[x][y][i][0], v1 = acc[x][y][i][1];
+            u32x4 pk;
+            pk[0] = op16<OT>::pack2_sat(v0[0] + bv[y][0].x, v0[1] + bv[y][0].y); pk[1] = op16<OT>::pack2_sat(v0[2] + bv[y][0].z, v0[3] + bv[y][0].w);
+            pk[2] = op16<OT>::pack2_sat(v1[0] + bv[y][1].x, v1[1] + bv[y][1].y); pk[3] = op16<OT>::pack2_sat(v1[2] + bv[y][1].z, v1[3] + bv[y][1].w);
+            if (t.sc1) __builtin_amdgcn_raw_buffer_store_b128(pk, rs_c, (m * t.ldc + n) * 2, 0, AUX_SC1);
+            else __builtin_amdgcn_raw_buffer_store_b128(pk, rs_c, (m * t.ldc + n) * 2, 0, 0);
+          }
+        }
+    };
+    if (chain) {
+      __builtin_amdgcn_sched_barrier(0);
+      asm volatile("buffer_inv sc0" ::: "memory");
+      ffp_stage_prologue(smem, ffp_tile_desc(a, n_type, n_u, n_nb));
+      __builtin_amdgcn_sched_barrier(0);
+      epilogue();
+      asm volatile("; staged" ::: "memory");
+    } else {
+      epilogue();
+    }
+    asm volatile("s_waitcnt vmcnt(0)" ::: "memory");
+    __syncthreads();
+    if (stats && wave == 0 && ffp_lane_id() == 0) ffp_stat(s_stat, type);
+    if (!chain) {
+      if (wave == 0 && ffp_lane_id() == 0) {
+        if (type == FF_JOB_L1) __hip_atomic_fetch_add(a.l1_cnt + u, 1u, __ATOMIC_RELAXED, __HIP_MEMORY_SCOPE_AGENT);
+        else {
+          const unsigned old = __hip_atomic_fetch_add(a.wih_cnt + u, 1u, __ATOMIC_RELAXED, __HIP_MEMORY_SCOPE_AGENT);
+          if (old + 1u == (unsigned)a.nt2)
+            __hip_atomic_fetch_add(a.gi_cnt + (u >> a.chunk_unit_shift), 1u, __ATOMIC_RELAXED, __HIP_MEMORY_SCOPE_AGENT);
+        }
+      }
+      return;
+    }
+    pub = true; p_wih = type == FF_JOB_WIH; p_u = u;
+    type = n_type; u = n_u; nb = n_nb; pre = true;
+  }
+}
+
+template <typename OT, bool IN16, typename PF>
 __device__ __forceinline__ void ffp_pack_rows(const FfPassArgs& a, int my_rows, int wave, int lane, const char* srgb, const char* sflow,
-                                              bf16_t* __restrict__ Xs) {
+                                              bf16_t* __restrict__ Xs, PF&& probe) {
   constexpr int ES = IN16 ? 2 : 4, NV = IN16 ? 1 : 2;
   constexpr int PR = 2;
   const int din = a.kx;
@@ -230,6 +458,7 @@
     issue(va, k + 2); PACK_FENCE();
     drain(vb, k + 1); PACK_FENCE();
   }
+  probe(); PACK_FENCE();
   if (k + 1 < n_rounds) {
     issue(vb, k + 1); PACK_FENCE();
     drain(va, k); PACK_FENCE();
@@ -240,8 +469,8 @@
 #undef PACK_FENCE
 }
 
-template <typename OT>
-__device__ __forceinline__ void ffp_pack(const FfPassArgs& a, int row0, int nrows, bf16_t* __restrict__ Xs) {
+template <typename OT, typename PF>
+__device__ __forceinline__ void ffp_pack(const FfPassArgs& a, int row0, int nrows, bf16_t* __restrict__ Xs, PF&& probe) {
   int tid_ = threadIdx.x;
   asm volatile("" : "+v"(tid_));
   const int lane = tid_ & 63, wave = __builtin_amdgcn_readfirstlane(tid_ >> 6);
@@ -268,14 +497,14 @@
     if (flow) sflow = (const char*)flow + (size_t)t * a.d_flow * es;
   }
   const int my_rows = nrows - wave * 32 < 32 ? nrows - wave * 32 : 32;
-  if (a.in16) ffp_pack_rows<OT, true>(a, my_rows, wave, lane, srgb, sflow, Xs);
-  else ffp_pack_rows<OT, false>(a, my_rows, wave, lane, srgb, sflow, Xs);
+  if (a.in16) ffp_pack_rows<OT, true>(a, my_rows, wave, lane, srgb, sflow, Xs, probe);
+  else ffp_pack_rows<OT, false>(a, my_rows, wave, lane, srgb, sflow, Xs, probe);
 }
 
 constexpr int FLN_MAX_E = 2048;
 
-template <typename OT, int NV, int NR>
-__device__ __forceinline__ void ffp_ln(const FfPassArgs& a, int nrows, const bf16_t* __restrict__ Ys, bf16_t* __restrict__ Es, const float* gb) {
+template <typename OT, int NV, int NR, typename PF>
+__device__ __forceinline__ void ffp_ln(const FfPassArgs& a, int nrows, const bf16_t* __restrict__ Ys, bf16_t* __restrict__ Es, const float* gb, PF&& probe) {
   int tid_ = threadIdx.x;
   asm volatile("" : "+v"(tid_));
   const int lane = tid_ & 63, wave = __builtin_amdgcn_readfirstlane(tid_ >> 6);
@@ -372,6 +601,7 @@
     request(ra, rb + 2 * STEP); LN_FENCE();
     process(rbuf, rb + STEP); LN_FENCE();
   }
+  probe(); LN_FENCE();
   if (rb + STEP < nrows) {
     request(rbuf, rb + STEP); LN_FENCE();
     process(ra, rb); LN_FENCE();
@@ -382,8 +612,8 @@
 #undef LN_FENCE
 }
 
-template <typename OT, int MAXV, int NR>
-__device__ __forceinline__ void ffp_ln_generic(const FfPassArgs& a, int nrows, const bf16_t* __restrict__ Ys, bf16_t* __restrict__ Es) {
+template <typename OT, int MAXV, int NR, typename PF>
+__device__ __forceinline__ void ffp_ln_generic(const FfPassArgs& a, int nrows, const bf16_t* __restrict__ Ys, bf16_t* __restrict__ Es, PF&& probe) {
   int tid_ = threadIdx.x;
   asm volatile("" : "+v"(tid_));
   const int lane = tid_ & 63, wave = tid_ >> 6;
@@ -403,6 +633,7 @@
   if (wave < nrows) request(raw, wave);
   for (int rb = wave; rb < nrows; rb += 8 * NR) {
     if (rb + 8 * NR < nrows) request(nxt, rb + 8 * NR);
+    else probe();
     auto unpack = [](const u32x4 w, float (&f)[8]) {
       f[0] = op16<OT>::lo(w[0]); f[1] = op16<OT>::hi(w[0]); f[2] = op16<OT>::lo(w[1]); f[3] = op16<OT>::hi(w[1]);
       f[4] = op16<OT>::lo(w[2]); f[5] = op16<OT>::hi(w[2]); f[6] = op16<OT>::lo(w[3]); f[7] = op16<OT>::hi(w[3]);
@@ -471,13 +702,13 @@
   }
 }
 
-template <typename OT>
-__device__ __forceinline__ void ffp_ln_any(const FfPassArgs& a, int nrows, const bf16_t* __restrict__ Ys, bf16_t* __restrict__ Es, const float* gb) {
+template <typename OT, typename PF>
+__device__ __forceinline__ void ffp_ln_any(const FfPassArgs& a, int nrows, const bf16_t* __restrict__ Ys, bf16_t* __restrict__ Es, const float* gb, PF&& probe) {
   switch (a.E >> 9) {
-    case 4: ffp_ln<OT, 4, 2>(a, nrows, Ys, Es, gb); break;
-    case 2: ffp_ln<OT, 2, 4>(a, nrows, Ys, Es, gb); break;
-    case 1: ffp_ln<OT, 1, 4>(a, nrows, Ys, Es, gb); break;
-    default: ffp_ln_generic<OT, 8, 2>(a, nrows, Ys, Es); break;
+    case 4: ffp_ln<OT, 4, 2>(a, nrows, Ys, Es, gb, probe); break;
+    case 2: ffp_ln<OT, 2, 4>(a, nrows, Ys, Es, gb, probe); break;
+    case 1: ffp_ln<OT, 1, 4>(a, nrows, Ys, Es, gb, probe); break;
+    default: ffp_ln_generic<OT, 8, 2>(a, nrows, Ys, Es, probe); break;
   }
 }
 
@@ -485,6 +716,8 @@
 __global__ __launch_bounds__(512, 2) void ff_pass_kernel(FfPassArgs a) {
   extern __shared__ __attribute__((aligned(16))) char smem[];
   __shared__ int s_job[2];
+  __shared__ int s_nx_[NX_WORDS];
+  int* s_nx = s_nx_;
   const int tid = threadIdx.x;
   const int xcc = __builtin_amdgcn_readfirstlane(__builtin_amdgcn_s_getreg((3 << 11) | 20) & 7);
   if (xcc < a.xcd_lo) return;
@@ -498,90 +731,91 @@
   __shared__ __attribute__((aligned(16))) float s_gb[2 * FLN_MAX_E];
   if (a.E <= FLN_MAX_E)
     for (int c = tid; c < a.E; c += 512) { s_gb[c] = a.ln_g[c]; s_gb[FLN_MAX_E + c] = a.ln_b[c]; }
-  const int q = xcc - a.xcd_lo, nf = 8 - a.xcd_lo;
-  const int n_q = a.n_units > q ? (a.n_units - q + nf - 1) / nf : 0;
-  const int sg = a.sg, tpr = sg * (2 + a.nt1 + a.nt2);
-  const int n_rounds = (n_q + sg - 1) / sg + a.lag3;
-  __shared__ unsigned long long s_stat[11];
+  __shared__ unsigned long long s_stat[FST_WORDS];
   const bool stats = a.stats != nullptr && tid == 0;
   if (stats) {
-    for (int e = 0; e < 8; ++e) s_stat[e] = 0;
-    s_stat[9] = __builtin_amdgcn_s_memrealtime(); s_stat[8] = s_stat[9]; s_stat[10] = __builtin_amdgcn_s_memtime();
-  }
-#define FSTAT(i) do { if (stats) { const unsigned long long n_ = __builtin_amdgcn_s_memrealtime(); s_stat[i] += n_ - s_stat[8]; s_stat[8] = n_; } } while (0)
+    for (int e = 0; e < FST_WORDS; ++e) s_stat[e] = 0;
+    s_stat[FST_T0] = __builtin_amdgcn_s_memrealtime(); s_stat[FST_LAST] = s_stat[FST_T0]; s_stat[FST_C0] = __builtin_amdgcn_s_memtime();
+  }
+#define FSTAT(i) do { if (stats) ffp_stat(s_stat, i); } while (0)
+  const bool look = a.lookahead != 0 && a.dbg == 0;
+  bool pre = false;
+  if (tid == 0) ffp_claim(a, s_nx);
   for (;;) {
     __syncthreads();
-    if (tid == 0) s_job[0] = (int)__hip_atomic_fetch_add(a.tick + q, 1u, __ATOMIC_RELAXED, __HIP_MEMORY_SCOPE_AGENT);
-    __syncthreads();
-    const int k = __builtin_amdgcn_readfirstlane(s_job[0]);
-    const int round = k / tpr, j = k - round * tpr;
+    const int state = __builtin_amdgcn_readfirstlane(s_nx[NX_STATE]);
+    const int type = __builtin_amdgcn_readfirstlane(s_nx[NX_TYPE]), u = __builtin_amdgcn_readfirstlane(s_nx[NX_UNIT]);
+    const int nb = __builtin_amdgcn_readfirstlane(s_nx[NX_NB]);
     FSTAT(5);
-    if (round >= n_rounds) break;
-    int type, i, nb = 0;
-    if (j < sg) { type = 0; i = round * sg + j; }
-    else if (j < sg + sg * a.nt1) { const int jj = j - sg; type = 1; nb = jj / sg; i = (round - a.lag1) * sg + (jj - nb * sg); }
-    else if (j < 2 * sg + sg * a.nt1) { type = 2; i = (round - a.lag2) * sg + (j - sg - sg * a.nt1); }
-    else { const int jj = j - 2 * sg - sg * a.nt1; type = 3; nb = jj / sg; i = (round - a.lag3) * sg + (jj - nb * sg); }
-    if (i < 0 || i >= n_q) continue;
-    const int u = q + i * nf;
+    if (state != NX_JOB) break;
+    const bool tile = type == FF_JOB_L1 || type == FF_JOB_WIH;
+    if (look) __syncthreads();
     if (tid == 0) {
+      if (look && !tile) ffp_claim(a, s_nx);
       bool ok = true;
-      const int up = u - a.ring_units;
-      if (type == 0) {
-        if (up >= 0) ok = ffp_wait_ge(a.l1_cnt + up, (unsigned)a.nt1, a.abort_word, 0x100u);
-      } else if (type == 1) {
-        ok = ffp_wait_ge(a.pack_done + u, 1u, a.abort_word, 0x101u);
-        if (ok && up >= 0) ok = ffp_wait_ge(a.ln_done + up, 1u, a.abort_word, 0x102u);
-      } else if (type == 2) {
-        ok = ffp_wait_ge(a.l1_cnt + u, (unsigned)a.nt1, a.abort_word, 0x103u);
-        if (ok && up >= 0) ok = ffp_wait_ge(a.wih_cnt + up, (unsigned)a.nt2, a.abort_word, 0x104u);
-      } else {
-        ok = ffp_wait_ge(a.ln_done + u, 1u, a.abort_word, 0x105u);
-        const int ug = u - a.gi_ring_units;
-        if (ok && ug >= 0) ok = ffp_wait_ge(a.rec_cnt + (ug >> a.chunk_unit_shift), (unsigned)a.rec_expect, a.abort_word, 0x106u);
+      if (!pre) {
+#pragma unroll
+        for (int e = 0; e < 2; ++e) {
+          FfWait w;
+          if (ok && ffp_job_wait(a, type, u, e, w)) ok = ffp_wait_ge(ffp_counter(a, w), ffp_need(a, w), a.abort_word, w.code);
+        }
       }
       s_job[1] = ok ? 1 : 0;
     }
     __syncthreads();
     if (!__builtin_amdgcn_readfirstlane(s_job[1])) break;
     FSTAT(4);
-    asm volatile("buffer_inv sc0" ::: "memory");
-    const int row0 = u * 256;
-    const int nrows = a.total_rows - row0 < 256 ? a.total_rows - row0 : 256;
-    const size_t slot = (size_t)(u % a.ring_units) * 256;
-    if (type == 0) {
-      if (!(a.dbg & 1)) ffp_pack<OT>(a, row0, nrows, a.X + slot * a.kx);
-    } else if (type == 1) {
-      if (!(a.dbg & 4))
-      ffp_tile<OT, false>(smem, a.X + slot * a.kx, a.kx, nrows, a.w1 + (size_t)nb * 256 * a.ld_w1, a.ld_w1, a.b1 + nb * 256,
-                          a.Y + slot * a.E + nb * 256, a.E, a.kx);
-    } else if (type == 2) {
-      if (a.dbg & 2) { }
-      else ffp_ln_any<OT>(a, nrows, a.Y + slot * a.E, a.Eb + slot * a.E, s_gb);
+    if (!pre) asm volatile("buffer_inv sc0" ::: "memory");
+    if (tile) {
+      if (!(a.dbg & (type == FF_JOB_L1 ? 4 : 8))) {
+        ffp_tiles<OT>(smem, a, s_nx, s_stat, type, u, nb, pre, look);
+      } else {
+        __syncthreads();
+        FSTAT(type);
+        if (tid == 0) {
+          if (type == FF_JOB_L1) __hip_atomic_fetch_add(a.l1_cnt + u, 1u, __ATOMIC_RELAXED, __HIP_MEMORY_SCOPE_AGENT);
+          else if (__hip_atomic_fetch_add(a.wih_cnt + u, 1u, __ATOMIC_RELAXED, __HIP_MEMORY_SCOPE_AGENT) + 1u == (unsigned)a.nt2)
+            __hip_atomic_fetch_add(a.gi_cnt + (u >> a.chunk_unit_shift), 1u, __ATOMIC_RELAXED, __HIP_MEMORY_SCOPE_AGENT);
+        }
+      }
+      pre = false;
     } else {
-      const size_t gslot = (size_t)(u & (a.gi_ring_units - 1)) * 256;
-      if (!(a.dbg & 8))
-      ffp_tile<OT, true>(smem, a.Eb + slot * a.E, a.E, nrows, a.w_ih + (size_t)nb * 256 * a.E, a.E, a.bias2 + nb * 256,
-                         a.GI + gslot * a.n3 + nb * 256, a.n3, a.E);
-    }
-    asm volatile("s_waitcnt vmcnt(0)" ::: "memory");
-    __syncthreads();
-    FSTAT(type);
-    if (tid == 0) {
-      if (type == 0) __hip_atomic_store(a.pack_done + u, 1u, __ATOMIC_RELAXED, __HIP_MEMORY_SCOPE_AGENT);
-      else if (type == 1) __hip_atomic_fetch_add(a.l1_cnt + u, 1u, __ATOMIC_RELAXED, __HIP_MEMORY_SCOPE_AGENT);
-      else if (type == 2) __hip_atomic_store(a.ln_done + u, 1u, __ATOMIC_RELAXED, __HIP_MEMORY_SCOPE_AGENT);
-      else {
-        const unsigned old = __hip_atomic_fetch_add(a.wih_cnt + u, 1u, __ATOMIC_RELAXED, __HIP_MEMORY_SCOPE_AGENT);
-        if (old + 1u == (unsigned)a.nt2)
-          __hip_atomic_fetch_add(a.gi_cnt + (u >> a.chunk_unit_shift), 1u, __ATOMIC_RELAXED, __HIP_MEMORY_SCOPE_AGENT);
-      }
-    }
+      const int row0 = u * 256;
+      const int nrows = a.total_rows - row0 < 256 ? a.total_rows - row0 : 256;
+      const size_t slot = (size_t)(u % a.ring_units) * 256;
+      auto probe = [&]() __attribute__((always_inline)) {
+        if (look && __builtin_amdgcn_readfirstlane(threadIdx.x >> 6) == 0) ffp_probe(a, s_nx);
+      };
+      if (type == FF_JOB_PACK) {
+        if (!(a.dbg & 1)) ffp_pack<OT>(a, row0, nrows, a.X + slot * a.kx, probe);
+      } else {
+        if (!(a.dbg & 2)) ffp_ln_any<OT>(a, nrows, a.Y + slot * a.E, a.Eb + slot * a.E, s_gb, probe);
+      }
+      if (stats) s_stat[FST_TILE_END] = 0;
+      bool staged = false;
+      if (look) {
+        ffp_bar_lds();
+        const int n_type = __builtin_amdgcn_readfirstlane(s_nx[NX_TYPE]);
+        staged = __builtin_amdgcn_readfirstlane(s_nx[NX_STATE]) == NX_JOB && __builtin_amdgcn_readfirstlane(s_nx[NX_READY]) != 0 &&
+                 (n_type == FF_JOB_L1 || n_type == FF_JOB_WIH);
+        if (staged) {
+          asm volatile("buffer_inv sc0" ::: "memory");
+          ffp_stage_prologue(smem, ffp_tile_desc(a, n_type, __builtin_amdgcn_readfirstlane(s_nx[NX_UNIT]), __builtin_amdgcn_readfirstlane(s_nx[NX_NB])));
+        }
+      }
+      asm volatile("s_waitcnt vmcnt(0)" ::: "memory");
+      __syncthreads();
+      FSTAT(type);
+      if (tid == 0) __hip_atomic_store((type == FF_JOB_PACK ? a.pack_done : a.ln_done) + u, 1u, __ATOMIC_RELAXED, __HIP_MEMORY_SCOPE_AGENT);
+      pre = staged;
+    }
+    if (!look && tid == 0) ffp_claim(a, s_nx);
   }
   if (stats) {
-    s_stat[7] = __builtin_amdgcn_s_memrealtime() - s_stat[9];
-    s_stat[6] = __builtin_amdgcn_s_memtime() - s_stat[10];
+    s_stat[7] = __builtin_amdgcn_s_memrealtime() - s_stat[FST_T0];
+    s_stat[6] = __builtin_amdgcn_s_memtime() - s_stat[FST_C0];
     for (int e = 0; e < 8; ++e) atomicAdd(a.stats + e, s_stat[e]);
+    atomicAdd(a.stats + 8, s_stat[FST_BETWEEN]); atomicAdd(a.stats + 9, s_stat[FST_BETWEEN_N]);
   }
 #undef FSTAT
 }
diff --git a/prego_amd/csrc/ff_ticket.h b/prego_amd/csrc/ff_ticket.h
--- /dev/null
+++ b/prego_amd/csrc/ff_ticket.h
@@ -0,0 +1,45 @@
+#pragma once
+
+enum { FF_JOB_PACK = 0, FF_JOB_L1 = 1, FF_JOB_LN = 2, FF_JOB_WIH = 3 };
+enum { FF_CNT_PACK = 0, FF_CNT_L1 = 1, FF_CNT_LN = 2, FF_CNT_WIH = 3, FF_CNT_REC = 4 };
+
+struct FfGeom {
+  int sg, nt1, nt2, lag1, lag2, lag3;
+};
+struct FfJob {
+  int round, type, i, nb;
+};
+struct FfWait {
+  int counter, index, need;
+  unsigned code;
+};
+
+__host__ __device__ inline int ff_tickets_per_round(const FfGeom& g) { return g.sg * (2 + g.nt1 + g.nt2); }
+__host__ __device__ inline int ff_queue_units(int n_units, int q, int nf) { return n_units > q ? (n_units - q + nf - 1) / nf : 0; }
+__host__ __device__ inline int ff_queue_rounds(int n_q, const FfGeom& g) { return (n_q + g.sg - 1) / g.sg + g.lag3; }
+
+__host__ __device__ inline FfJob ff_ticket_decode(int k, const FfGeom& g) {
+  const int sg = g.sg, tpr = ff_tickets_per_round(g);
+  FfJob b;
+  b.round = k / tpr;
+  b.nb = 0;
+  const int j = k - b.round * tpr;
+  if (j < sg) { b.type = FF_JOB_PACK; b.i = b.round * sg + j; }
+  else if (j < sg + sg * g.nt1) { const int jj = j - sg; b.type = FF_JOB_L1; b.nb = jj / sg; b.i = (b.round - g.lag1) * sg + (jj - b.nb * sg); }
+  else if (j < 2 * sg + sg * g.nt1) { b.type = FF_JOB_LN; b.i = (b.round - g.lag2) * sg + (j - sg - sg * g.nt1); }
+  else { const int jj = j - 2 * sg - sg * g.nt1; b.type = FF_JOB_WIH; b.nb = jj / sg; b.i = (b.round - g.lag3) * sg + (jj - b.nb * sg); }
+  return b;
+}
+
+__host__ __device__ inline bool ff_job_wait(int type, int u, const FfGeom& g, int ring_units, int gi_ring_units, int chunk_unit_shift, int which,
+                                            FfWait& w) {
+  const int up = u - ring_units;
+  const int ug = u - gi_ring_units;
+  const bool own = which == 0 && type != FF_JOB_PACK;
+  const bool have = own || (type == FF_JOB_PACK ? which == 0 && up >= 0 : which == 1 && (type == FF_JOB_WIH ? ug >= 0 : up >= 0));
+  if (type == FF_JOB_PACK) w = FfWait{FF_CNT_L1, up, g.nt1, 0x100u};
+  else if (type == FF_JOB_L1) w = own ? FfWait{FF_CNT_PACK, u, 1, 0x101u} : FfWait{FF_CNT_LN, up, 1, 0x102u};
+  else if (type == FF_JOB_LN) w = own ? FfWait{FF_CNT_L1, u, g.nt1, 0x103u} : FfWait{FF_CNT_WIH, up, g.nt2, 0x104u};
+  else w = own ? FfWait{FF_CNT_LN, u, 1, 0x105u} : FfWait{FF_CNT_REC, ug >> chunk_unit_shift, 0, 0x106u};
+  return have;
+}
diff --git a/prego_amd/csrc/kernels.h b/prego_amd/csrc/kernels.h
--- a/prego_amd/csrc/kernels.h
+++ b/prego_amd/csrc/kernels.h
@@ -95,6 +95,7 @@
   int max_wg;
   int lag1, lag2, lag3;
   int dbg;
+  int lookahead;
   unsigned long long* stats;
   int f16;
   unsigned* tick;
diff --git a/prego_amd/csrc/miniroad.cpp b/prego_amd/csrc/miniroad.cpp
--- a/prego_amd/csrc/miniroad.cpp
+++ b/prego_amd/csrc/miniroad.cpp
@@ -132,7 +132,7 @@
   }
   if (e == hipSuccess) e = hipEventCreateWithFlags(&h->ev_fork, hipEventDisableTiming);
   if (e == hipSuccess) e = hipEventCreateWithFlags(&h->ev_join, hipEventDisableTiming);
-  A((void**)&h->stamps, 8 * sizeof(unsigned long long));
+  A((void**)&h->stamps, 16 * sizeof(unsigned long long));
   A((void**)&h->tile_ctr, 4096 * sizeof(unsigned));
   if (e == hipSuccess) e = hipHostMalloc((void**)&h->pin_place, 64, hipHostMallocDefault);
   if (e == hipSuccess) e = hipEventCreateWithFlags(&h->ev_place, hipEventDisableTiming);
@@ -143,7 +143,7 @@
   h->xcd_overlap = getenv("PREGO_NO_XCD_OVERLAP") == nullptr;
   if (const char* sp = getenv("PREGO_SPLIT_PASS")) h->chooser.split_env = atoi(sp);
   A((void**)&h->st_scratch, (size_t)16 * ((size_t)emb * 6 + (size_t)3 * H * 8));
-  if (e == hipSuccess) e = hipMemset(h->stamps, 0, 8 * sizeof(unsigned long long));
+  if (e == hipSuccess) e = hipMemset(h->stamps, 0, 16 * sizeof(unsigned long long));
   h->use_stamps = prego_tune_env("PREGO_GRU_STAMPS") != nullptr;
   if (e == hipSuccess) e = hipMemset(h->hx, 0, h->x2 ? gru_x2_hx_bytes(H, h->G) : gru_hx_bytes(h->bf16, H, h->G));
   if (e == hipSuccess) e = hipMemset(h->flags, 0, ((size_t)h->G * h->P + 16) * sizeof(unsigned));
diff --git a/prego_amd/csrc/miniroad_handle.h b/prego_amd/csrc/miniroad_handle.h
--- a/prego_amd/csrc/miniroad_handle.h
+++ b/prego_amd/csrc/miniroad_handle.h
@@ -95,6 +95,7 @@
   const float* peer_guard = nullptr;
   unsigned* pin_hs = nullptr; unsigned hs_seq = 0;
   int dbg_fault = 0;
+  int dbg_lookahead = 1;
   hipEvent_t ev_split[4] = {nullptr, nullptr, nullptr, nullptr};
   double split_rec_ms = 0, split_ff_ms = 0; long long split_passes = 0, split_steps = 0; bool split_ev_pending = false;
   std::string err;
diff --git a/prego_amd/csrc/miniroad_split.cpp b/prego_amd/csrc/miniroad_split.cpp
--- a/prego_amd/csrc/miniroad_split.cpp
+++ b/prego_amd/csrc/miniroad_split.cpp
@@ -1,4 +1,5 @@
 #include "miniroad_handle.h"
+#include "ff_ticket.h"
 
 #include <algorithm>
 #include <chrono>
@@ -114,6 +115,9 @@
 #ifdef PREGO_DEBUG_ABI
   static const int dbg = prego_tune_env("PREGO_SPLIT_DBG") ? atoi(prego_tune_env("PREGO_SPLIT_DBG")) : 0;
   fa.dbg = dbg;
+  fa.lookahead = (h->dbg_lookahead && !dbg) ? 1 : 0;
+#else
+  fa.lookahead = 1;
 #endif
   fa.tick = tick; fa.pack_done = pack_done; fa.l1_cnt = l1_cnt; fa.ln_done = ln_done; fa.wih_cnt = wih_cnt; fa.gi_cnt = gi_cnt;
   fa.rec_cnt = rec_cnt; fa.abort_word = h->abort_word; fa.hs = hs;
@@ -207,4 +211,45 @@
   h->dbg_fault = mode;
   return PREGO_OK;
 }
+
+extern "C" int prego_debug_split_lookahead(prego_miniroad* h, int on) {
+  if (!h) return prego_fail_(PREGO_EINVAL, "debug split lookahead: handle is NULL");
+  h->dbg_lookahead = on ? 1 : 0;
+  return PREGO_OK;
+}
+
+extern "C" int prego_debug_split_stats(prego_miniroad* h, unsigned long long* out10) {
+  if (!h || !out10) return prego_fail_(PREGO_EINVAL, "debug split stats: NULL");
+  HIPCHK(hipDeviceSynchronize());
+  HIPCHK(hipMemcpy(out10, h->stamps, 10 * sizeof(unsigned long long), hipMemcpyDeviceToHost));
+  HIPCHK(hipMemset(h->stamps, 0, 10 * sizeof(unsigned long long)));
+  return PREGO_OK;
+}
+
+extern "C" int prego_debug_ff_ticket(int k, int n_units, int nf, int q, int sg, int nt1, int nt2, int lag1, int lag2, int lag3, int ring_units,
+                                     int gi_ring_units, int chunk_unit_shift, int32_t* out16) {
+  if (!out16 || k < 0 || n_units < 1 || nf < 1 || nf > 7 || q < 0 || q >= nf || sg < 1 || nt1 < 1 || nt2 < 1 || chunk_unit_shift < 0)
+    return prego_fail_(PREGO_EINVAL, "debug ff ticket: arguments");
+  const FfGeom g{sg, nt1, nt2, lag1, lag2, lag3};
+  const int n_q = ff_queue_units(n_units, q, nf);
+  const FfJob b = ff_ticket_decode(k, g);
+  for (int e = 0; e < 16; ++e) out16[e] = 0;
+  out16[1] = b.round; out16[2] = b.type; out16[3] = b.i; out16[4] = b.nb;
+  if (b.round >= ff_queue_rounds(n_q, g)) { out16[0] = 2; return PREGO_OK; }
+  if (b.i < 0 || b.i >= n_q) { out16[0] = 1; return PREGO_OK; }
+  const int u = q + b.i * nf;
+  out16[5] = u;
+  int n = 0;
+  for (int e = 0; e < 2; ++e) {
+    FfWait w;
+    if (!ff_job_wait(b.type, u, g, ring_units, gi_ring_units, chunk_unit_shift, e, w)) continue;
+    out16[7 + 3 * n] = w.counter; out16[8 + 3 * n] = w.index; out16[9 + 3 * n] = w.need;
+    ++n;
+  }
+  out16[6] = n;
+  out16[13] = b.type;
+  out16[14] = u;
+  out16[15] = b.type == FF_JOB_L1 ? nt1 : b.type == FF_JOB_WIH ? nt2 : 1;
+  return PREGO_OK;
+}
 #endif
```

Result: slower. 19.71 million frames/s (-21.2%).
